# Cogito2012/OpenTAL

Hardware: AMD Instinct MI355X
Metric: clips/sec training step, 256-frame THUMOS14 clips (higher is better)
Workload: dtype bf16

## Files before the change

include/opental_hip.h:

```cpp
#ifndef OPENTAL_HIP_H
#define OPENTAL_HIP_H

#include <stdint.h>
#include <stddef.h>

#ifdef __cplusplus
extern "C" {
#endif

#define OTAL_ABI_VERSION 26

#define OTAL_E_NULL      (-1)
#define OTAL_E_SHAPE     (-2)
#define OTAL_E_ODD_C     (-3)
#define OTAL_E_BATCH     (-4)
#define OTAL_E_DTYPE     (-5)
#define OTAL_E_LEVELS    (-6)
#define OTAL_E_UNSUPPORTED (-7)

#define OTAL_F32  0
#define OTAL_BF16 1
#define OTAL_F16  2
#define OTAL_F64  3

#define OTAL_MAX_LEVELS 8

int otal_abi_version(void);
const char* otal_error_string(int code);
int otal_set_option(const char* name, int value);
int otal_get_option(const char* name, int dflt);
int otal_stream_wait(void* waiter, void* signaler);

int otal_bmp_fwd(const void* in, const float* seg, void* out,
                 int B, int C, int T, int N, int seg_batch, int dtype, void* stream);

int otal_bmp_bwd(const void* grad_out, const void* in, const float* seg, void* grad_in,
                 int B, int C, int T, int N, int seg_batch, int compat_ref_stride,
                 int dtype, void* stream);

int otal_bmp_fwd_levels(const void* in, const float* seg, void* out,
                        int B, int C, int nlev, const int* t_start, const int* n_start,
                        int dtype, void* stream);
int otal_bmp_bwd_levels(const void* grad_out, const void* in, const float* seg, void* grad_in,
                        int B, int C, int nlev, const int* t_start, const int* n_start,
                        int dtype, void* stream);

int otal_conv_half_storage(const int* geom, const int64_t* strides, int mode, int precision);
size_t otal_conv_workspace_bytes(const int* geom, int mode);

int otal_conv_fwd(const int* geom, const int64_t* strides, const float* x, const float* w,
                  const float* scale, const float* shift, float* y, int relu, int precision,
                  const void* prologue, void* ws, size_t ws_bytes, void* stream);

int otal_conv_dgrad(const int* geom, const int64_t* strides, const float* dy, const float* wt_packed,
                    float* dx, int accumulate, const float* out_mask, const float* out_scale,
                    int precision, const void* prologue, void* ws, size_t ws_bytes, void* stream);

int otal_conv_wgrad(const int* geom, const int64_t* strides, const float* x, const float* dy,
                    float* dw, int accumulate, int precision, const void* prologue, void* ws, size_t ws_bytes,
                    void* stream);

int otal_conv_fwd_pair(const int* geom, const int64_t* strides, const float* const* x, const float* const* w,
                       const float* const* scale, const float* const* shift, float* const* y, int relu, int precision,
                       const void* const* prologue, void* ws, size_t ws_bytes, void* stream);
int otal_conv_dgrad_pair(const int* geom, const int64_t* strides, const float* const* dy, const float* const* w,
                         float* const* dx, int precision, const void* const* prologue, void* ws, size_t ws_bytes, void* stream);
int otal_conv_wgrad_pair(const int* geom, const int64_t* strides, const float* const* x, const float* const* dy,
                         float* const* dw, int precision, void* ws, size_t ws_bytes, void* stream);

size_t otal_conv_prologue_bytes(const int* geom, const int64_t* strides, int mode, int precision);
size_t otal_conv_prologue_desc_bytes(void);
int otal_conv_prologue(const int* geom, const int64_t* strides, int mode, const float* w, int precision, void* region,
                       size_t region_bytes, void* host_desc, void* stream);
int otal_conv_prologue_batch(int n, const void* device_descs, const int* device_starts, int total_blocks, void* stream);

int otal_conv_defer_reduces(int on);
size_t otal_conv_deferred_end(void);
int otal_conv_deferred_count(void);
int otal_conv_flush_reduces(void* stream);

const char* otal_conv_last_kernel(void);

int otal_conv_pack_wt(const float* w, float* wt, int Cout, int Cin, int kvol, void* stream);

int otal_gn_relu_fwd(const float* x, const float* gamma, const float* beta, float* y, float* stats,
                     int B, int C, int T, int G, float eps, int relu, int nlev, const int* lev, void* stream);
int otal_gn_relu_bwd(const float* dy, int64_t dy_batch_stride, const float* x, const float* gamma, const float* beta,
                     const float* stats, float* dx, float* partial, int B, int C, int T, int G,
                     int relu, int nlev, const int* lev, void* stream);
int otal_gn_relu_fwd_pair(const float* const* x, const float* const* gamma, const float* const* beta, float* const* y,
                          float* const* stats, int B, int C, int T, int G, float eps, int relu, int nlev, const int* lev,
                          void* stream);
int otal_gn_relu_bwd_pair(const float* const* dy, const int64_t* dy_batch_stride, const float* const* x,
                          const float* const* gamma, const float* const* beta, const float* const* stats, float* const* dx,
                          float* const* partial, int B, int C, int T, int G, int relu, int nlev, const int* lev, void* stream);
int otal_sum_partials(int n_items, const float* const* partial, float* const* dst0, float* const* dst1,
                      float* const* dst2, const int* channels, const int* batches, void* stream);

const char* otal_layer_last_kernel(void);

int otal_maxpool3d_fwd(const int* geom, const int64_t* strides, const float* x, float* y,
                       unsigned char* argtap, void* stream);
int otal_maxpool3d_bwd(const int* geom, const int64_t* strides, const float* dy,
                       const unsigned char* argtap, float* dx, int accumulate,
                       const float* out_mask, const float* out_scale, void* stream);
size_t otal_maxpool3d_signbits_bytes(const int* geom, const int64_t* strides);
int otal_maxpool3d_fwd_signbits(const int* geom, const int64_t* strides, const float* x, float* y,
                                unsigned char* argtap, unsigned char* signbits, void* stream);
int otal_maxpool3d_bwd_signbits(const int* geom, const int64_t* strides, const float* dy, const unsigned char* argtap,
                                float* dx, int accumulate, const unsigned char* signbits, const float* out_scale,
                                void* stream);
int otal_maxpool3d_fwd_signbits_h(const int* geom, const int64_t* strides, const void* x_bf16, float* y,
                                  unsigned char* argtap, unsigned char* signbits, void* stream);
int otal_maxpool3d_bwd_signbits_h(const int* geom, const int64_t* strides, const float* dy, const unsigned char* argtap,
                                  void* dx_bf16, const unsigned char* signbits, const float* out_scale, void* stream);
int otal_maxpool3d_fwd_io(const int* geom, const int64_t* strides, const void* x, void* y, unsigned char* argtap,
                          unsigned char* signbits, int io, void* stream);
int otal_maxpool3d_bwd_io(const int* geom, const int64_t* strides, const void* dy, const unsigned char* argtap, void* dx,
                          int accumulate, const void* out_mask, const float* out_scale, const unsigned char* signbits, int io,
                          void* stream);
int otal_convert_storage(const void* src, int64_t src_bs, int64_t src_cs, void* dst, int64_t dst_bs, int64_t dst_cs,
                         int to_bf16, int B, int C, int P, void* stream);

int otal_head_outputs_fwd(int n_items, const int* channels, const int* modes, const float* const* raw, float* const* out,
                          float* const* unct, const float* scales, int B, int N, int nlev, const int* lev,
                          const float* level_strides, void* stream);
int otal_head_outputs_bwd(int n_items, const int* channels, const int* modes, const float* const* raw,
                          const float* const* out, const float* const* unct, const float* const* dout,
                          const float* const* dunct, float* const* draw, const float* scales, float* dscales, int B,
                          int N, int nlev, const int* lev, const float* level_strides, void* stream);

int otal_boundary_bce(const float* x, int64_t x_batch_stride, int64_t x_channel_stride, const float* mask,
                      int64_t mask_batch_stride, int64_t mask_row_stride, int mask_row0, int mask_step, float* terms,
                      float* dx, int B, int C, int T, void* stream);

int otal_boundary_finish(int n, const float* const* terms, const float* weights, const int* T, int B, float* out2, void* stream);
int otal_boundary_scale(int n, const float* const* dx, float* const* out, const float* weights, const int* C, const int* T,
                        int B, const float* g_start, const float* g_end, void* stream);

int otal_proposal_windows(const float* loc, float* seg, float* frame_seg, int B, int nlev,
                          const int* lev, float frame_num, void* stream);

int otal_decode_clips(const float* loc, const float* prop_loc, const float* priors, const float* conf,
                      const float* prop_conf, const float* center, const float* act, const float* prop_act,
                      const float* offsets, const float* fps, float* seg, float* score, float* unct,
                      float* actn, unsigned char* flag, int nclips, int A, int K, float clip_length,
                      float conf_thresh, void* stream);
int otal_decode_clips_ex(const float* loc, const float* prop_loc, const float* priors, const float* conf,
                         const float* prop_conf, const float* center, const float* act, const float* prop_act,
                         const float* offsets, const float* fps, float* seg, float* score, float* unct,
                         float* actn, unsigned char* flag, int nclips, int A, int K, float clip_length,
                         float conf_thresh, int score_fn, int first_class, void* stream);
int otal_decode_clips_ev(const float* loc, const float* prop_loc, const float* priors, const float* conf,
                         const float* prop_conf, const float* center, const float* act, const float* prop_act,
                         const float* offsets, const float* fps, float* seg, float* score, float* unct,
                         float* actn, unsigned char* flag, int nclips, int A, int K, float clip_length,
                         float conf_thresh, int score_fn, int first_class, int evidence, void* stream);
int otal_softnms_classes(const float* seg, const float* score, const float* unct, const float* actn,
                         const unsigned char* flag, const int* clip_start, int nvideos, int max_clips,
                         int A, int K, float sigma, int top_k, float score_threshold, float* out,
                         int* counts, int* out_index, int out_cols, void* stream);
size_t otal_softnms_scratch_bytes(int total_clips, int max_clips, int A, int K);
int otal_softnms_classes_ws(const float* seg, const float* score, const float* unct, const float* actn,
                            const unsigned char* flag, const int* clip_start, int nvideos, int max_clips,
                            int A, int K, float sigma, int top_k, float score_threshold, float* out,
                            int* counts, int* out_index, int out_cols, void* scratch, size_t scratch_bytes,
                            int total_clips, void* stream);
int otal_detection_table(const float* rows, const int* counts, const double* durations, int V, int K, int top_k, int cols,
                         int drop_empty, int scoring, int* video, int* cls, double* seg, float* sup, double* known,
                         int* list_start, void* stream);
int otal_anchor_stats(const float* loc, const float* conf, const float* prop_conf, const float* center, const float* act,
                      const float* prop_act, const float* priors, const float* gt, const unsigned char* gvalid, int B, int K,
                      int C, int G, float clip_length, float overlap_thresh, int os_head, int n_known, int target,
                      int score_bins, int grad_bins, long long* hist_score, long long* hist_grad, int* label, float* value,
                      float* grad, void* stream);
int otal_anchor_stats_ev(const float* loc, const float* conf, const float* prop_conf, const float* center, const float* act,
                         const float* prop_act, const float* priors, const float* gt, const unsigned char* gvalid, int B,
                         int K, int C, int G, float clip_length, float overlap_thresh, int os_head, int n_known, int target,
                         int score_bins, int grad_bins, long long* hist_score, long long* hist_grad, int* label,
                         float* value, float* grad, int evidence, void* stream);

int otal_openmax_dist(const float* feat, int N, int rows_per_batch, int64_t sb, int64_t sr, int64_t sc, const float* mav,
                      int K, int D, const int* labels, float* dist, void* stream);
int otal_openmax_class_means(const float* feat, int N, int rows_per_batch, int64_t sb, int64_t sr, int64_t sc,
                             const int* labels, int K, int D, float* means, int* counts, void* stream);
int otal_openmax_probs(const float* logits, int64_t ldl, const float* feat, int N, int rows_per_batch, int64_t sb, int64_t sr,
                       int64_t sc, const float* mav, const float* wb, int K, int D, int R, float* probs, void* stream);
int otal_decode_clips_openmax(const float* loc, const float* prop_loc, const float* priors, const float* conf,
                              const float* prop_conf, const float* center, const float* offsets, const float* fps,
                              const float* feat, const float* prop_feat, const int64_t* feat_strides,
                              const int64_t* prop_feat_strides, const float* mav, const float* mav_prop, const float* wb,
                              const float* wb_prop, float* seg, float* score, float* unknown, unsigned char* flag,
                              int nclips, int A, int C, int first_class, int D, int R, int refined_feature,
                              float clip_length, float conf_thresh, void* stream);

int otal_openmax_dist_wide(const float* feat, int N, int rows_per_batch, int64_t sb, int64_t sr, int64_t sc, const float* mav,
                           int K, int D, const int* labels, float* dist, void* stream);
int otal_openmax_probs_wide(const float* logits, int64_t ldl, const float* feat, int N, int rows_per_batch, int64_t sb,
                            int64_t sr, int64_t sc, const float* mav, const float* wb, int K, int D, int R, float* probs,
                            void* stream);
int otal_decode_clips_openmax_wide(const float* loc, const float* prop_loc, const float* priors, const float* conf,
                                   const float* prop_conf, const float* center, const float* offsets, const float* fps,
                                   const float* feat, const float* prop_feat, const int64_t* feat_strides,
                                   const int64_t* prop_feat_strides, const float* mav, const float* mav_prop, const float* wb,
                                   const float* wb_prop, float* seg, float* score, float* unknown, unsigned char* flag,
                                   int nclips, int A, int C, int first_class, int D, int R, int refined_feature,
                                   float clip_length, float conf_thresh, void* stream);

int otal_head_convs_supported(int n_heads, int n_inputs, const int* in_idx, const int* cout, const int* ksize, int B, int C, int N);
int otal_head_convs_fwd(int n_heads, int n_inputs, const int* in_idx, const int* cout, const int* ksize,
                        const float* const* x, const float* const* w, const float* const* bias, float* const* y, int B, int C,
                        int N, int nlev, const int* lev, void* stream);
int otal_head_convs_bwd(int n_heads, int n_inputs, const int* in_idx, const int* cout, const int* ksize,
                        const float* const* x, const float* const* w, const float* const* dy, float* const* dx,
                        float* const* dw, float* const* db, int B, int C, int N, int nlev, const int* lev, void* stream);
int otal_head_convs_bwd_parts(int n_heads, int n_inputs, const int* in_idx, const int* cout, const int* ksize,
                        const float* const* x, const float* const* w, const float* const* dy, float* const* dx,
// ... 116 lines not shown
```

opental_amd/common/ops.py:

```python
import bisect
import ctypes
import os
import warnings
from typing import NamedTuple

import torch

from .. import _lib as L
from .conv_geom import make_geom

_WORKSPACE = {}
WORKSPACE_BYTES = 192 << 20
WORKSPACE_TOTAL = 512 << 20

CONV_PROFILE = None

CONV_PRECISION = 0
HALF_STORAGE = os.environ.get("OTAL_HALF_STORAGE", "1") != "0"
HALF_ACT_DIRECT = os.environ.get("OTAL_HALF_ACT_DIRECT", "0") != "0"
HALF_CHAIN = os.environ.get("OTAL_HALF_CHAIN", "1") != "0"


def _prof_begin():
    if CONV_PROFILE is None:
# ... 527 lines not shown

def _prologue(mode, ga, sa, pkey, w, prec):
    c = STEP.prologues
    if c is None or not (prec & 1):
        return None
    wp = 0
    if mode != 2:
        wp = w.data_ptr()
        r = c.persistent_range
        if r is None or not (r[0] <= wp < r[1]):
            return None
    reg = c.region(mode, ga, sa, (wp, pkey, prec), w, prec)
    if reg is None:
        return None
    return L.ptr(reg)


_PLANS = {}


def _plan(mode, xs, ys, Cout, k, s, levels, spatial_valid, xname, yname):
    key = (mode, xs.shape, xs.stride(), ys.shape, ys.stride(), Cout, k, s, levels, spatial_valid, xs.dtype, ys.dtype,
           xs.device, ys.device)
    plan = _PLANS.get(key)
    if plan is None:
        x5, y5 = _as5(xs), _as5(ys)
        B, Cin, Ti, Hi, Wi = x5.shape
        g, outn = _make_geom(B, Cin, Cout, (Ti, Hi, Wi), k, s, levels, spatial_valid)
        if tuple(y5.shape) != (B, Cout) + outn:
            raise RuntimeError(f"{yname} has shape {tuple(y5.shape)}, expected {(B, Cout) + outn}")
        _check(x5, xname, x5.dtype)
        _check(y5, yname, y5.dtype)
        ga, sa = _geom_arrays(g, x5, y5)
        plan = (g, ga, sa, (mode, tuple(g), _bs(x5), _bs(y5)), (tuple(x5.shape), _bs(x5)))
        if len(_PLANS) > 4096:
            _PLANS.clear()
        _PLANS[key] = plan
    return plan


def _out_positions(x, Cout, k, s, levels, spatial_valid):
    x5 = _as5(x)
    B, Cin, Ti, Hi, Wi = x5.shape
    return _make_geom(B, Cin, Cout, (Ti, Hi, Wi), k, s, levels, spatial_valid)[1]


def half_storage_ok(mode, x_shape, cout, k, s, both=False):
    if not (HALF_STORAGE and int(CONV_PRECISION) & 1) or len(x_shape) != 5:
        return False
    k, s = _k3(k), _k3(s)
    B, Cin, Ti, Hi, Wi = x_shape
    g, outn = _make_geom(B, Cin, cout, (Ti, Hi, Wi), k, s, None, False)
    ga = (ctypes.c_int * len(g))(*g)
    P = outn[0] * outn[1] * outn[2]
    sa = (ctypes.c_int64 * 4)(Cin * Ti * Hi * Wi, Ti * Hi * Wi, cout * P, P)
    return bool(L.lib().otal_conv_half_storage(ga, sa, int(mode), int(CONV_PRECISION) | (12 if both else 0)))


def conv_forward(x, w, k, s, scale=None, shift=None, relu=False, spatial_valid=False, levels=None, out=None, half_out=False):
    k, s = _k3(k), _k3(s)
    if levels is not None:
        levels = tuple(levels)
    Cout = w.shape[0]
    if x.dtype == torch.bfloat16:
        return _conv_forward_half(x, w, k, s, scale, shift, relu, spatial_valid, levels, out)
    if out is None:
        outn = _out_positions(x, Cout, k, s, levels, spatial_valid)
        out = torch.empty((x.shape[0], Cout) + (outn if x.dim() == 5 else outn[:1]),
                          dtype=torch.bfloat16 if half_out else x.dtype, device=x.device)
    if out.dtype != (torch.bfloat16 if half_out else torch.float32) or x.dtype != torch.float32:
        raise RuntimeError("conv_forward: float32 tensors (bfloat16 y with half_out)")
    g, ga, sa, pkey, _ = _plan(0, x, out, Cout, k, s, levels, spatial_valid, "x", "y")
    if not w.is_contiguous():
        raise RuntimeError("weights must be contiguous")
    wsp, wsn = _ws_args(x.device)
    ev = _prof_begin()
    prec = int(CONV_PRECISION)
    pre = _prologue(0, ga, sa, pkey, w, prec)
    L.check(L.lib().otal_conv_fwd(ga, sa, L.ptr(x), L.ptr(w), _opt(scale), _opt(shift), L.ptr(out), int(relu),
                                  prec | (4 if half_out else 0), pre, wsp, wsn, L.stream()),
            "otal_conv_fwd")
    _prof_end(ev, "fwd", g)
    return out


def _conv_forward_half(x, w, k, s, scale, shift, relu, spatial_valid, levels, out):
    Cout = w.shape[0]
    if out is None:
        outn = _out_positions(x, Cout, k, s, levels, spatial_valid)
        out = torch.empty((x.shape[0], Cout) + (outn if x.dim() == 5 else outn[:1]), dtype=torch.bfloat16, device=x.device)
    if out.dtype != torch.bfloat16 or not (int(CONV_PRECISION) & 1):
        raise RuntimeError("conv_forward: a bfloat16 x needs a bfloat16 y and the bf16-operand mode")
    g, ga, sa, pkey, _ = _plan(0, x, out, Cout, k, s, levels, spatial_valid, "x", "y")
    if not w.is_contiguous():
        raise RuntimeError("weights must be contiguous")
    wsp, wsn = _ws_args(x.device)
    ev = _prof_begin()
    prec = int(CONV_PRECISION)
    pre = _prologue(0, ga, sa, pkey, w, prec)
    L.check(L.lib().otal_conv_fwd(ga, sa, L.ptr(x), L.ptr(w), _opt(scale), _opt(shift), L.ptr(out), int(relu),
                                  prec | 12, pre, wsp, wsn, L.stream()), "otal_conv_fwd (bf16 tensors)")
    _prof_end(ev, "fwd", g)
    return out


def pack_wt(w):
    Cout, Cin = w.shape[0], w.shape[1]
    kvol = w[0, 0].numel()
    wt = torch.empty((Cin, Cout, kvol), dtype=w.dtype, device=w.device)
    L.check(L.lib().otal_conv_pack_wt(L.ptr(w), L.ptr(wt), Cout, Cin, kvol, L.stream()), "otal_conv_pack_wt")
    return wt


def conv_dgrad(dy, w, x_shape, k, s, spatial_valid=False, levels=None, out=None,
               accumulate=False, wt=None, out_mask=None, out_scale=None):
    k, s = _k3(k), _k3(s)
    if levels is not None:
        levels = tuple(levels)
    Cout = w.shape[0]
    if out is None:
        if accumulate:
            raise RuntimeError("accumulate needs an existing buffer")
        out = torch.empty(tuple(x_shape), dtype=dy.dtype, device=dy.device)
    elif tuple(out.shape) != tuple(x_shape):
        raise RuntimeError(f"conv_dgrad: out has shape {tuple(out.shape)}, expected {tuple(x_shape)}")
    half = dy.dtype == torch.bfloat16
    if out.dtype != dy.dtype or not (half or dy.dtype == torch.float32):
        raise RuntimeError("conv_dgrad: float32 tensors, or bfloat16 dy / dx / out_mask together")
    if half and (accumulate or not (int(CONV_PRECISION) & 1)):
        raise RuntimeError("conv_dgrad: bfloat16 tensors need the bf16-operand mode and a plain store")
    g, ga, sa, pkey, xlay = _plan(1, out, dy, Cout, k, s, levels, spatial_valid, "dx", "dy")
    prec = int(CONV_PRECISION)
    if wt is None:
        wt = w if w.is_contiguous() else w.contiguous()
        prec |= 2
    wsp, wsn = _ws_args(dy.device)
    ev = _prof_begin()
    if out_mask is not None:
        m5 = _as5(out_mask)
        if (tuple(m5.shape), _bs(m5)) != xlay or out_mask.dtype != dy.dtype:
            raise RuntimeError("out_mask must share dx's shape, layout and dtype")
    pre = _prologue(1, ga, sa, pkey, wt, prec) if (prec & 2) else None
    if half:
        prec |= 12 | (16 if out_mask is not None else 0)
    L.check(L.lib().otal_conv_dgrad(ga, sa, L.ptr(dy), L.ptr(wt), L.ptr(out),
                                    int(accumulate), _opt(out_mask), _opt(out_scale), prec, pre,
                                    wsp, wsn, L.stream()),
            "otal_conv_dgrad")
    _prof_end(ev, "dgrad", g)
    return out


def is_full_collapse(x_shape, k, s, spatial_valid):
    return (spatial_valid and len(x_shape) == 5 and tuple(x_shape[3:]) == tuple(k[1:]) and k[0] == 1
            and tuple(s) == (1, 1, 1))


def conv_dgrad_collapse(dy, w, x_shape):
    B, Cin, T, H, W = x_shape
    Cout = w.shape[0]
    wa = w.detach().reshape(1, Cout, Cin * H * W)
    dyt = dy.reshape(B, Cout, T).permute(0, 2, 1).reshape(B * T, Cout, 1).contiguous()
    dxp = conv_forward(wa, dyt, 1, 1)
    return dxp.view(B, T, Cin, H, W).permute(0, 2, 1, 3, 4)


# ... 168 lines not shown
def conv_wgrad_pair(xs, dys, w_shape, k, s, levels=None, outs=(None, None)):
    k, s = _k3(k), _k3(s)
    if levels is not None:
        levels = tuple(levels)
    if not PAIR_LAUNCHES or not (int(CONV_PRECISION) & 1) or not _same_layout(xs[0], xs[1]) or not _same_layout(dys[0], dys[1]):
        return None
    if xs[0].dtype != torch.float32 or dys[0].dtype != torch.float32:
        return None
    Cout = w_shape[0]
    g, ga, sa, pkey, _ = _plan(2, xs[0], dys[0], Cout, k, s, levels, False, "x", "dy")
    outs = [o if o is not None else torch.empty(tuple(w_shape), dtype=torch.float32, device=xs[0].device) for o in outs]
    if not (outs[0].is_contiguous() and outs[1].is_contiguous()):
        return None
    st = STEP
    if st.defer and st.defer_owner is not None and st.defer_owner[0] != st.ws_index:
        flush_reduces()
    wsp, wsn = _ws_args(xs[0].device)
    ev = _prof_begin()
    rc = L.lib().otal_conv_wgrad_pair(ga, sa, _pp(*xs), _pp(*dys), _pp(*outs), int(CONV_PRECISION), wsp, wsn, L.stream())
    if rc == L.E_UNSUPPORTED:
        return None
    L.check(rc, "otal_conv_wgrad_pair")
    if st.defer:
        _after_wgrad(xs[0].device)
    _prof_end(ev, "wgrad", g, 2)
    return outs


def gn_relu_forward_pair(xs, gammas, betas, groups=32, eps=1e-5, relu=True, levels=None, outs=None):
    if not PAIR_LAUNCHES or not _same_layout(xs[0], xs[1]) or not xs[0].is_contiguous():
        return None
    L.require_device(*xs, *gammas, *betas)
    B, C, T = xs[0].shape
    nlev, lev = _lev_arg(levels)
    stats = [torch.empty((B, groups, nlev, 2), dtype=torch.float32, device=x.device) for x in xs]
    if outs is not None:
        st0, st1 = _dest_strides(outs[0], B, C, T), _dest_strides(outs[1], B, C, T)
        if st0 != st1:
            return None
        rc = L.lib().otal_gn_relu_fwd_pair_to(_pp(*xs), _pp(*gammas), _pp(*betas), _pp(*outs), ctypes.c_int64(st0[0]),
                                              ctypes.c_int64(st0[1]), _pp(*stats), B, C, T, groups, ctypes.c_float(eps), int(relu),
                                              nlev, lev, L.stream())
        if rc == L.E_UNSUPPORTED:
            return None
        L.check(rc, "otal_gn_relu_fwd_pair_to")
        return list(zip(outs, stats))
    ys = [torch.empty_like(x) for x in xs]
    rc = L.lib().otal_gn_relu_fwd_pair(_pp(*xs), _pp(*gammas), _pp(*betas), _pp(*ys), _pp(*stats), B, C, T, groups,
                                       ctypes.c_float(eps), int(relu), nlev, lev, L.stream())
    if rc == L.E_UNSUPPORTED:
        return None
    L.check(rc, "otal_gn_relu_fwd_pair")
    return list(zip(ys, stats))


def _lev_arg(levels):
    if levels is None or len(levels) <= 2:
        return 1, None
    return len(levels) - 1, L.int_array(list(levels))


def _dest_strides(out, B, C, T):
    if tuple(out.shape) != (B, C, T) or out.dtype != torch.float32 or not out.is_cuda or (T > 1 and out.stride(2) != 1):
        raise RuntimeError("gn_relu_forward: `out` must be a float32 (B,C,T) GPU tensor with dense positions")
    cs = out.stride(1) if C > 1 else T
    return (out.stride(0) if B > 1 else cs * C), cs


def gn_relu_forward(x, gamma, beta, groups=32, eps=1e-5, relu=True, levels=None, out=None):
    L.require_device(x, gamma, beta)
    B, C, T = x.shape
    nlev, lev = _lev_arg(levels)
    stats = torch.empty((B, groups, nlev, 2), dtype=torch.float32, device=x.device)
    if out is not None:
        bs, cs = _dest_strides(out, B, C, T)
        L.check(L.lib().otal_gn_relu_fwd_to(L.ptr(x), L.ptr(gamma), L.ptr(beta), L.ptr(out), ctypes.c_int64(bs), ctypes.c_int64(cs),
                                            L.ptr(stats), B, C, T, groups, ctypes.c_float(eps), int(relu), nlev, lev, L.stream()),
                "otal_gn_relu_fwd_to")
        return out, stats
    y = torch.empty_like(x)
    L.check(L.lib().otal_gn_relu_fwd(L.ptr(x), L.ptr(gamma), L.ptr(beta), L.ptr(y), L.ptr(stats), B, C, T, groups,
                                     ctypes.c_float(eps), int(relu), nlev, lev, L.stream()), "otal_gn_relu_fwd")
    return y, stats


def pyramid_merge_forward(p0, p1, total, up):
    L.require_device(p0, p1)
    B, C, t0 = p0.shape
    if tuple(p1.shape) != (B, C, t0 // 2):
        raise RuntimeError("pyramid_merge_forward: p1 must have half of p0's positions")
    packed = torch.empty((B, C, total), dtype=torch.float32, device=p0.device)
    frame = torch.empty((B, C, t0 * up), dtype=torch.float32, device=p0.device)
    L.check(L.lib().otal_pyramid_merge_fwd(L.ptr(p0), L.ptr(p1), L.ptr(packed), L.ptr(frame), B, C, t0, total, up, L.stream()),
            "otal_pyramid_merge_fwd")
    return packed, frame


def pyramid_merge_backward(da, db, dframe, dnext, t0, up):
    L.require_device(da, dframe)
    B, C, T = da.shape
    dp0 = torch.empty((B, C, t0), dtype=torch.float32, device=da.device)
    dp1 = torch.empty((B, C, t0 // 2), dtype=torch.float32, device=da.device)
    for t in (db, dnext):
        if t is not None:
            L.require_device(t)
    L.check(L.lib().otal_pyramid_merge_bwd(L.ptr(da), _opt(db), L.ptr(dframe), _opt(dnext), L.ptr(dp0), L.ptr(dp1), B, C, t0, T, up,
                                           L.stream()), "otal_pyramid_merge_bwd")
    return dp0, dp1


def gn_relu_backward(dy, x, gamma, beta, stats, groups=32, relu=True, levels=None, bias=None):
    B, C, T = x.shape
    if dy.dim() != 3 or tuple(dy.shape) != (B, C, T) or dy.stride(2) != 1 or dy.stride(1) != T or dy.stride(0) < C * T:
        dy = dy.contiguous()
    L.require_device(x, gamma, beta, stats)
    if not dy.is_cuda:
        raise RuntimeError("opental_amd ops run on the GPU only")
    nlev, lev = _lev_arg(levels)
    dx = torch.empty_like(x)
    partial = torch.empty((B, 3, C), dtype=torch.float32, device=x.device)
    L.check(L.lib().otal_gn_relu_bwd(L.ptr(dy), ctypes.c_int64(dy.stride(0)), L.ptr(x), L.ptr(gamma), L.ptr(beta), L.ptr(stats),
                                     L.ptr(dx), L.ptr(partial), B, C, T, groups, int(relu), nlev, lev, L.stream()),
            "otal_gn_relu_bwd")
    return (dx,) + _gn_sums(partial, gamma, beta, bias, C, B)


def _gn_sums(partial, gamma, beta, bias, C, B):
    s = STEP
    if s.pending_sums is not None and bias is not None and s.slots is not None:
        slots = [s.slots.take(t) for t in (gamma, beta, bias)]
        if all(sl is not None for sl in slots):
            s.pending_sums.append((partial, tuple(sl.data_ptr() for sl in slots), C, B))
            return slots[0], slots[1], slots[2]
        for t, sl in zip((gamma, beta, bias), slots):
            if sl is not None:
                s.slots.release(t)
    red = partial.sum(0)
    return red[0], red[1], red[2]


def gn_relu_backward_pair(dys, xs, gammas, betas, stats, groups=32, relu=True, levels=None, biases=(None, None)):
    if not PAIR_LAUNCHES or not _same_layout(xs[0], xs[1]):
        return None
    B, C, T = xs[0].shape
    dys = list(dys)
    for i in range(2):
        dy = dys[i]
        if dy.dim() != 3 or tuple(dy.shape) != (B, C, T) or dy.stride(2) != 1 or dy.stride(1) != T or dy.stride(0) < C * T:
            dys[i] = dy.contiguous()
        if not dys[i].is_cuda:
            raise RuntimeError("opental_amd ops run on the GPU only")
    L.require_device(*xs, *gammas, *betas, *stats)
    nlev, lev = _lev_arg(levels)
    dxs = [torch.empty_like(x) for x in xs]
    partials = [torch.empty((B, 3, C), dtype=torch.float32, device=x.device) for x in xs]
    rc = L.lib().otal_gn_relu_bwd_pair(_pp(*dys), (ctypes.c_int64 * 2)(dys[0].stride(0), dys[1].stride(0)), _pp(*xs), _pp(*gammas),
                                       _pp(*betas), _pp(*stats), _pp(*dxs), _pp(*partials), B, C, T, groups, int(relu), nlev, lev,
                                       L.stream())
    if rc == L.E_UNSUPPORTED:
        return None
    L.check(rc, "otal_gn_relu_bwd_pair")
    return [(dxs[i],) + _gn_sums(partials[i], gammas[i], betas[i], biases[i], C, B) for i in range(2)]


def flush_pending_sums():
    items = STEP.pending_sums
# ... 240 lines not shown
    @staticmethod
    def backward(ctx, *gs):
        (grads,) = ctx.saved_tensors
        B, K, C = ctx.dims
        A = B * K
        gs = [None if g is None else g.contiguous() for g in gs]
        out = torch.empty(4 * A + 2 * A * C + 3 * A, dtype=torch.float32, device=grads.device)
        g7 = (ctypes.c_void_p * 7)(*[None if g is None else g.data_ptr() for g in gs])
        L.check(L.lib().otal_detection_loss_bwd(L.ptr(grads), g7, L.ptr(out), B, K, C, L.stream()), "otal_detection_loss_bwd")
        o = 0
        def take(n, shape):
            nonlocal o
            v = out[o:o + n].view(shape)
            o += n
            return v
        d_loc, d_pl = take(2 * A, (B, K, 2)), take(2 * A, (B, K, 2))
        d_conf, d_pconf = take(A * C, (B, K, C)), take(A * C, (B, K, C))
        d_cen, d_act, d_pact = take(A, (B, K)), take(A, (B, K)), take(A, (B, K))
        heads = tuple(d if there else None for d, there in zip((d_loc, d_conf, d_pl, d_pconf, d_cen, d_act, d_pact), ctx.heads))
        return heads + (None,) * (len(ctx.needs_input_grad) - len(heads))


class DetectionLossFunction(_FusedLossFunction):
    ENTRIES = {'plain': 'otal_detection_loss', 'ex': 'otal_detection_loss_ex', 'ev': 'otal_detection_loss_ev'}
    TERMS = 7

    @staticmethod
    def c_args(call, state, B, K, C, G):
        args = [L.ptr(state), B, K, C, G, *_cf(call.clip_length, call.overlap_thresh), int(call.ibm_active), int(call.num_bins),
                *_cf(call.momentum), int(call.iou_aware), int(call.cls_mode), *_cf(call.focal_alpha)]
        if call.entry != 'plain':
            args += [int(call.reweight), *_cf(call.rw_gamma)]
        if call.entry == 'ev':
            args += [int(call.evidence), int(call.loss_type)]
        return args, L.lib().otal_detection_loss_scratch_floats(B, K)


class AnetDetectionLossFunction(_FusedLossFunction):
    ENTRIES = {'anet_ex': 'otal_detection_loss_anet_ex', 'anet_ev': 'otal_detection_loss_anet_ev'}
    TERMS = 7

    @staticmethod
    def c_args(call, state, B, K, C, G):
        nlev = len(call.level_bounds)
        lbs = (ctypes.c_float * (2 * nlev))(*[float(v) for row in call.level_bounds for v in row])
        args = [B, K, C, G, *_cf(call.clip_length, call.overlap_thresh), lbs, nlev, int(call.ibm_active), *_cf(call.ibm_coeff),
                int(call.iou_aware), *_cf(call.act_weight, call.act_margin), int(call.cls_mode), *_cf(call.focal_alpha)]
        if call.entry == 'anet_ev':
            args += [int(call.evidence), int(call.loss_type)]
        return args, 8 * B


class RPLDetectionLossFunction(_FusedLossFunction):
    ENTRIES = {'rpl': 'otal_detection_loss_rpl'}
    TERMS = 5

    @staticmethod
    def c_args(call, state, B, K, C, G):
        args = [B, K, C, G, *_cf(call.clip_length, call.overlap_thresh), int(bool(call.gcpl)),
                *_cf(call.temperature, call.weight_pl, call.radius)]
        return args, L.lib().otal_detection_loss_scratch_floats(B, K)


_SLOT_INDEX = {}


def _adjacent_view(ts):
    if not ts or any(t is None or t.numel() != 1 or t.dtype != torch.float32 for t in ts):
        return None
    base = ts[0]
    st = base.untyped_storage().data_ptr()
    if any(t.untyped_storage().data_ptr() != st or t.data_ptr() != base.data_ptr() + 4 * i for i, t in enumerate(ts)):
        return None
    return base.detach().as_strided((len(ts),), (1,), base.storage_offset())


class HeadOutputsFunction(torch.autograd.Function):

    @staticmethod
    def forward(ctx, levels, level_strides, modes, *tensors):
        nlev_ = len(levels) - 1
        ctx.scale_params = tensors[:nlev_]
        scales = _adjacent_view(tensors[:nlev_])
        if scales is None:
            scales = torch.cat([t.detach().reshape(1) for t in tensors[:nlev_]])
        raws = [r.contiguous() for r in tensors[nlev_:]]
        L.require_device(scales, *raws)
        B, _, N = raws[0].shape
        n = len(raws)
        outs = [torch.empty((B, N, r.shape[1]), dtype=torch.float32, device=r.device) for r in raws]
        uncts = [torch.empty((B, N), dtype=torch.float32, device=raws[0].device) if m >= 2 else None for m in modes]
        VP = ctypes.c_void_p * n
        arr = lambda ts: VP(*[None if t is None else t.data_ptr() for t in ts])
        strides = None if level_strides is None else (ctypes.c_float * len(level_strides))(*level_strides)
        meta = (L.int_array([r.shape[1] for r in raws]), L.int_array(list(modes)), len(levels) - 1, L.int_array(list(levels)), strides, B, N, n)
        L.check(L.lib().otal_head_outputs_fwd(n, meta[0], meta[1], arr(raws), arr(outs), arr(uncts), L.ptr(scales), B, N, meta[2],
                                              meta[3], strides, L.stream()), "otal_head_outputs_fwd")
        ctx.meta, ctx.modes = meta, tuple(modes)
        ctx.save_for_backward(scales, *raws, *outs, *[u for u in uncts if u is not None])
        return tuple(outs) + tuple(u for u in uncts if u is not None)

    @staticmethod
    def backward(ctx, *grads):
        chans, modes_a, nlev, lev, strides, B, N, n = ctx.meta
        saved = ctx.saved_tensors
        scales, raws, outs, us = saved[0], saved[1:1 + n], saved[1 + n:1 + 2 * n], list(saved[1 + 2 * n:])
        uncts, dunct, k = [], [], 0
        for m in ctx.modes:
            if m >= 2:
                uncts.append(us[k]); dunct.append(grads[n + k]); k += 1
            else:
                uncts.append(None); dunct.append(None)
        douts = [None if g is None else g.contiguous() for g in grads[:n]]
        dunct = [None if g is None else g.contiguous() for g in dunct]
        draws = [torch.empty_like(r) for r in raws]
        VP = ctypes.c_void_p * n
        arr = lambda ts: VP(*[None if t is None else t.data_ptr() for t in ts])

        def launch(dscales):
            L.check(L.lib().otal_head_outputs_bwd(n, chans, modes_a, arr(raws), arr(outs), arr(uncts), arr(douts), arr(dunct), arr(draws),
                                                  L.ptr(scales), L.ptr(dscales), B, N, nlev, lev, strides, L.stream()),
                    "otal_head_outputs_bwd")
        want = all(ctx.needs_input_grad[3:3 + nlev])
        slots = [grad_slot(p) if want else None for p in ctx.scale_params]
        direct = _adjacent_view(slots) if all(sl is not None for sl in slots) else None
        if direct is not None:
            direct.zero_()
            launch(direct)
            return (None, None, None) + tuple(slots) + tuple(draws)
        dscales = torch.zeros_like(scales)
        launch(dscales)
        if all(sl is not None for sl in slots):
            key = tuple(sl.data_ptr() for sl in slots)
            idx = _SLOT_INDEX.get(key)
            if idx is None:
                flat = STEP.slots.grad
                idx = torch.tensor([(sl.data_ptr() - flat.data_ptr()) // 4 for sl in slots], dtype=torch.int64).to(flat.device)
                if len(_SLOT_INDEX) > 64:
                    _SLOT_INDEX.clear()
                _SLOT_INDEX[key] = idx
            STEP.slots.grad.index_copy_(0, idx, dscales)
            return (None, None, None) + tuple(slots) + tuple(draws)
        for p, sl in zip(ctx.scale_params, slots):
            if sl is not None:
                STEP.slots.release(p)
        aligned = torch.zeros((nlev, 4), dtype=dscales.dtype, device=dscales.device)
        aligned[:, 0] = dscales
        return (None, None, None) + tuple(aligned[l, :1] for l in range(nlev)) + tuple(draws)


def _hc_meta(heads, n_inputs):
    n = len(heads)
    return (n, n_inputs, L.int_array([h[0] for h in heads]), L.int_array([h[1] for h in heads]), L.int_array([h[2] for h in heads]))


def head_convs_supported(heads, n_inputs, B, C, N):
    if not 1 <= len(heads) <= 8 or not 1 <= n_inputs <= 4:
        return False
    n, ni, idx, co, ks = _hc_meta(heads, n_inputs)
    return bool(L.lib().otal_head_convs_supported(n, ni, idx, co, ks, int(B), int(C), int(N)))


class HeadConvsFunction(torch.autograd.Function):

    @staticmethod
    def forward(ctx, levels, heads, n_inputs, *tensors):
        nh = len(heads)
        xs = [t.contiguous() for t in tensors[:n_inputs]]
        ws = list(tensors[n_inputs:n_inputs + nh])
        bs = list(tensors[n_inputs + nh:n_inputs + 2 * nh])
        L.require_device(*xs, *ws, *[b for b in bs if b is not None])
        B, C, N = xs[0].shape
        spec = [(heads[i][0], int(ws[i].shape[0]), int(heads[i][1])) for i in range(nh)]
        for (j, co, k), w in zip(spec, ws):
            if tuple(w.shape) != (co, C, k) or tuple(xs[j].shape) != (B, C, N) or w.dtype != torch.float32:
                raise RuntimeError("head_convs: weight / input shapes do not match")
        meta = _hc_meta(spec, n_inputs)
        nlev, lev = _lev_arg(levels)
        ys = [torch.empty((B, co, N), dtype=torch.float32, device=xs[0].device) for _, co, _ in spec]
        VP = lambda ts: (ctypes.c_void_p * len(ts))(*[None if t is None else t.data_ptr() for t in ts])
        L.check(L.lib().otal_head_convs_fwd(*meta, VP(xs), VP(ws), VP(bs), VP(ys), B, C, N, nlev, lev, L.stream()),
                "otal_head_convs_fwd")
        ctx.cfg = (meta, nlev, lev, n_inputs, nh, (B, C, N), [b is not None for b in bs])
        ctx.bias_params = bs
        ctx.save_for_backward(*xs, *ws)
        return tuple(ys)

    @staticmethod
    def backward(ctx, *dys):
        meta, nlev, lev, n_inputs, nh, (B, C, N), has_bias = ctx.cfg
        saved = ctx.saved_tensors
        xs, ws = list(saved[:n_inputs]), list(saved[n_inputs:])
        dys = [None if g is None else g.contiguous() for g in dys]
        dxs = [torch.empty_like(x) if ctx.needs_input_grad[3 + j] else None for j, x in enumerate(xs)]
        dws, slots_w, slots_b = [], [], []
        for w in ws:
            slot = grad_slot(w)
            slots_w.append(slot)
            dws.append(slot if slot is not None else torch.empty_like(w))
        dbs = []
        for w, b in zip(ws, ctx.bias_params):
            slot = grad_slot(b) if b is not None else None
            slots_b.append(slot)
            dbs.append(slot if slot is not None else (torch.empty(w.shape[0], dtype=torch.float32, device=w.device) if b is not None else None))
        VP = lambda ts: (ctypes.c_void_p * len(ts))(*[None if t is None else t.data_ptr() for t in ts])
        in_slots = all(s_ is not None for s_ in slots_w) and all(s_ is not None for s_, b in zip(slots_b, ctx.bias_params) if b is not None)
        side = side_wgrads(xs[0].device)
        if side.on and in_slots and STEP.defer_join:
            L.check(L.lib().otal_head_convs_bwd_parts(*meta, VP(xs), VP(ws), VP(dys), VP(dxs), VP(dws), VP(dbs), B, C, N, nlev, lev, 1,
                                                      L.stream()), "otal_head_convs_bwd_parts")
            dst_w, dst_b = [t.detach() for t in dws], [None if t is None else t.detach() for t in dbs]
            side.pending.append(lambda: L.check(L.lib().otal_head_convs_bwd_parts(
                *meta, VP(xs), VP(ws), VP(dys), VP([None] * len(xs)), VP(dst_w), VP(dst_b), B, C, N, nlev, lev, 2, L.stream()),
# ... 47 lines not shown
            side.node_end(True)
        else:
            run(opt(dx), L.ptr(dcen), 3 if dx is not None else 2)
        return dx, dcen


def head_convs(levels, items):
    maps, heads = [], []
    for x, unit in items:
        j = next((i for i, m in enumerate(maps) if m is x), None)
        if j is None:
            j = len(maps)
            maps.append(x)
        conv = unit.conv1d
        k = conv.kernel_size[0]
        if conv.stride[0] != 1 or k not in (1, 3) or x.dim() != 3 or x.dtype != torch.float32 or not x.is_cuda:
            return None
        heads.append((j, k, conv))
    B, C, N = maps[0].shape
    if any(tuple(m.shape) != (B, C, N) for m in maps) or C % 16:
        return None
    if not head_convs_supported([(j, conv.out_channels, k) for j, k, conv in heads], len(maps), B, C, N):
        return None
    return HeadConvsFunction.apply(None if levels is None else tuple(levels), tuple((j, k) for j, k, _ in heads), len(maps),
                                   *maps, *[c.weight for _, _, c in heads], *[c.bias for _, _, c in heads])


HC_MAX_ROWS = 21


def head_convs_mixed(levels, items, run_one):
    wide = [unit.conv1d.out_channels > HC_MAX_ROWS for _, unit in items]
    if not any(wide) or all(wide):
        return None
    small = [it for it, w in zip(items, wide) if not w]
    fused = head_convs(levels, small)
    if fused is None:
        return None
    fused = list(fused)
    return [run_one(x, unit) if w else fused.pop(0) for (x, unit), w in zip(items, wide)]


class BoundaryBCEFunction(torch.autograd.Function):

    @staticmethod
    def forward(ctx, x, mask, row0, step):
        if not (x.is_cuda and mask.is_cuda):
            raise RuntimeError("opental_amd ops run on the GPU only")
        B, C, T = x.shape
        if x.stride(2) != 1 or mask.stride(2) != 1 or x.dtype != torch.float32 or mask.dtype != torch.float32:
            raise RuntimeError("boundary_bce: float32 maps with unit time stride")
        if row0 + 2 > mask.shape[1] or (T - 1) * step >= mask.shape[2]:
            raise RuntimeError("boundary_bce: mask rows / length do not cover the map")
        terms = torch.empty((B, 2, T), dtype=torch.float32, device=x.device)
        dx = torch.empty((B, C, T), dtype=torch.float32, device=x.device)
        L.check(L.lib().otal_boundary_bce(L.ptr(x), ctypes.c_int64(x.stride(0)), ctypes.c_int64(x.stride(1)), L.ptr(mask),
                                          ctypes.c_int64(mask.stride(0)), ctypes.c_int64(mask.stride(1)), int(row0), int(step),
                                          L.ptr(terms), L.ptr(dx), B, C, T, L.stream()), "otal_boundary_bce")
        ctx.save_for_backward(dx)
        ctx.x_shape = tuple(x.shape)
        losses = terms.sum(dim=(0, 2)) / float(B * T)
        return losses[0], losses[1]

    @staticmethod
    def backward(ctx, g_start, g_end):
        (dx,) = ctx.saved_tensors
        B, C, T = ctx.x_shape
        z = dx.new_zeros(())
        g = torch.stack([z if g_start is None else g_start.reshape(()), z if g_end is None else g_end.reshape(())])
        return (dx.view(B, 2, C // 2, T) * g.view(1, 2, 1, 1)).view(B, C, T), None, None, None


class BoundaryLossesFunction(torch.autograd.Function):

    @staticmethod
    def forward(ctx, mask, steps, weights, *xs):
        n = len(xs)
        B = xs[0].shape[0]
        terms, dxs = [], []
        for x, step in zip(xs, steps):
            if not (x.is_cuda and mask.is_cuda) or x.stride(2) != 1 or mask.stride(2) != 1 or x.dtype != torch.float32:
                raise RuntimeError("boundary losses: float32 GPU maps with unit time stride")
            _, C, T = x.shape
            if 2 > mask.shape[1] or (T - 1) * step >= mask.shape[2]:
                raise RuntimeError("boundary losses: mask rows / length do not cover the map")
            t = torch.empty((B, 2, T), dtype=torch.float32, device=x.device)
            dx = torch.empty((B, C, T), dtype=torch.float32, device=x.device)
            L.check(L.lib().otal_boundary_bce(L.ptr(x), ctypes.c_int64(x.stride(0)), ctypes.c_int64(x.stride(1)), L.ptr(mask),
                                              ctypes.c_int64(mask.stride(0)), ctypes.c_int64(mask.stride(1)), 0, int(step),
                                              L.ptr(t), L.ptr(dx), B, C, T, L.stream()), "otal_boundary_bce")
            terms.append(t); dxs.append(dx)
        out = torch.empty(2, dtype=torch.float32, device=xs[0].device)
        wa = (ctypes.c_float * n)(*[float(w) for w in weights])
        VP = lambda ts: (ctypes.c_void_p * n)(*[t.data_ptr() for t in ts])
        L.check(L.lib().otal_boundary_finish(n, VP(terms), wa, L.int_array([t.shape[2] for t in terms]), B, L.ptr(out), L.stream()),
                "otal_boundary_finish")
        ctx.save_for_backward(*dxs)
        ctx.meta = (n, B, [float(w) for w in weights])
        return out[0], out[1]

    @staticmethod
    def backward(ctx, g_start, g_end):
        dxs = ctx.saved_tensors
        n, B, weights = ctx.meta
        outs = [torch.empty_like(d) for d in dxs]
        wa = (ctypes.c_float * n)(*weights)
        VP = lambda ts: (ctypes.c_void_p * n)(*[t.data_ptr() for t in ts])
        gs = [None if g is None else g.contiguous() for g in (g_start, g_end)]
        L.check(L.lib().otal_boundary_scale(n, VP(dxs), VP(outs), wa, L.int_array([d.shape[1] for d in dxs]),
                                            L.int_array([d.shape[2] for d in dxs]), B, _opt(gs[0]), _opt(gs[1]), L.stream()),
                "otal_boundary_scale")
        return (None, None, None) + tuple(outs)


def eval_match(pred_seg, pred_start, gt_seg, gt_start, thresholds):
    L.require_device(pred_seg, pred_start, gt_seg, gt_start, thresholds)
    if pred_seg.dtype != torch.float64 or gt_seg.dtype != torch.float64 or thresholds.dtype != torch.float64 \
            or pred_start.dtype != torch.int32 or gt_start.dtype != torch.int32:
        raise RuntimeError("eval_match: segments and thresholds in float64, offsets in int32")
    if pred_seg.dim() != 2 or pred_seg.shape[1] != 2 or gt_seg.dim() != 2 or gt_seg.shape[1] != 2 \
            or pred_start.dim() != 1 or pred_start.shape != gt_start.shape or pred_start.numel() < 1 or thresholds.dim() != 1:
        raise RuntimeError("eval_match: pred_seg (N, 2), gt_seg (M, 2), pred_start / gt_start (ngroups + 1), thresholds (nthr,)")
    N, ngroups, nthr = pred_seg.shape[0], pred_start.numel() - 1, thresholds.numel()
    out = torch.empty((nthr, N), dtype=torch.int32, device=pred_seg.device)
    nonfinite = torch.zeros(1, dtype=torch.int32, device=pred_seg.device)
    if N == 0 or ngroups == 0:
        return out, nonfinite
    if gt_seg.shape[0] == 0:
        gt_seg = gt_seg.new_zeros((1, 2))
    L.check(L.lib().otal_eval_match(L.ptr(pred_seg), L.ptr(pred_start), L.ptr(gt_seg), L.ptr(gt_start), L.ptr(thresholds),
                                    ngroups, nthr, L.ptr(out), L.ptr(nonfinite), L.stream()), "otal_eval_match")
    return out, nonfinite


def eval_match_labeled(pred_seg, pred_label, pred_start, gt_seg, gt_label, gt_start, thresholds):
    L.require_device(pred_seg, pred_label, pred_start, gt_seg, gt_label, gt_start, thresholds)
    if pred_seg.dtype != torch.float64 or gt_seg.dtype != torch.float64 or thresholds.dtype != torch.float64 \
            or any(t.dtype != torch.int32 for t in (pred_start, gt_start, pred_label, gt_label)):
        raise RuntimeError("eval_match_labeled: segments and thresholds in float64, offsets and labels in int32")
    if pred_seg.dim() != 2 or pred_seg.shape[1] != 2 or gt_seg.dim() != 2 or gt_seg.shape[1] != 2 \
            or pred_start.dim() != 1 or pred_start.shape != gt_start.shape or pred_start.numel() < 1 or thresholds.dim() != 1 \
            or pred_label.shape != pred_seg.shape[:1] or gt_label.shape != gt_seg.shape[:1]:
        raise RuntimeError("eval_match_labeled: pred_seg (N, 2), pred_label (N), gt_seg (M, 2), gt_label (M), "
                           "pred_start / gt_start (ngroups + 1), thresholds (nthr,)")
    N, ngroups, nthr = pred_seg.shape[0], pred_start.numel() - 1, thresholds.numel()
    out = torch.empty((nthr, N), dtype=torch.int32, device=pred_seg.device)
    max_tiou = torch.zeros(N, dtype=torch.float64, device=pred_seg.device)
    nonfinite = torch.zeros(1, dtype=torch.int32, device=pred_seg.device)
    if N == 0 or ngroups == 0:
        return out, max_tiou, nonfinite
    if gt_seg.shape[0] == 0:
        gt_seg, gt_label = gt_seg.new_zeros((1, 2)), gt_label.new_zeros(1)
    L.check(L.lib().otal_eval_match_labeled(L.ptr(pred_seg), L.ptr(pred_label), L.ptr(pred_start), L.ptr(gt_seg), L.ptr(gt_label),
                                            L.ptr(gt_start), L.ptr(thresholds), ngroups, nthr, L.ptr(out), L.ptr(max_tiou),
                                            L.ptr(nonfinite), L.stream()), "otal_eval_match_labeled")
    return out, max_tiou, nonfinite


AP_TILE = 256
AP_MAX_CLASS_ROWS = 2 ** 31 - 1 - AP_TILE


def average_precision(codes, rank_pos, class_start, gt_count, out=None):
    L.require_device(codes, rank_pos, class_start, gt_count)
    if any(t.dtype != torch.int32 for t in (codes, rank_pos, class_start, gt_count)):
        raise RuntimeError("average_precision: codes, rank_pos, class_start and gt_count in int32")
    if codes.dim() != 2 or rank_pos.dim() != 1 or rank_pos.shape[0] != codes.shape[1] or class_start.dim() != 1 \
            or class_start.numel() < 2 or gt_count.dim() != 1 or gt_count.numel() != class_start.numel() - 1:
        raise RuntimeError("average_precision: codes (nthr, N), rank_pos (N), class_start (K + 1), gt_count (K)")
    nthr, N = codes.shape
    K = gt_count.numel()
    if out is None:
        out = torch.empty((nthr, K), dtype=torch.float64, device=codes.device)
    else:
        L.require_device(out)
        if tuple(out.shape) != (nthr, K) or out.dtype != torch.float64:
            raise RuntimeError("average_precision: out must be (nthr, K) float64")
# ... 110 lines not shown
```

opental_amd/csrc/bce.hip:

```cpp
#include "common.h"

namespace {

__global__ __launch_bounds__(256) void boundary_bce_kernel(const float* __restrict__ x, int64_t x_bs, int64_t x_cs,
                                                           const float* __restrict__ mask, int64_t m_bs, int64_t m_rs, int row0,
                                                           int m_step, float* __restrict__ terms, float* __restrict__ dx,
                                                           int B, int C, int T) {
    __shared__ float part[16][17];
    const int tl = threadIdx.x & 15, cg = threadIdx.x >> 4;
    const int t = blockIdx.x * 16 + tl, b = blockIdx.y, h = blockIdx.z;
    const int half = C >> 1;
    const bool live = t < T;
    const float* xp = x + (int64_t)b * x_bs + (int64_t)h * half * x_cs + (live ? t : 0);
    constexpr int BCE_MAXI = 32;
    float th[BCE_MAXI];
    const int nit = live ? (half - cg + 15) / 16 : 0;
    float s = 0.f;
#pragma unroll
    for (int i0 = 0; i0 < BCE_MAXI; i0 += 8) {
        if (i0 >= nit) { for (int u = 0; u < 8; ++u) th[i0 + u] = 0.f; continue; }
        float v[8];
#pragma unroll
        for (int u = 0; u < 8; ++u) v[u] = xp[(int64_t)(cg + 16 * min(i0 + u, max(nit - 1, 0))) * x_cs];
#pragma unroll
        for (int u = 0; u < 8; ++u) {
            th[i0 + u] = tanhf(v[u]);
            if (i0 + u < nit) s += th[i0 + u];
        }
    }
    for (int i = BCE_MAXI; i < nit; ++i) s += tanhf(xp[(int64_t)(cg + 16 * i) * x_cs]);
    part[cg][tl] = s;
    __syncthreads();
    float tot = 0.f;
#pragma unroll
    for (int k = 0; k < 16; ++k) tot += part[k][tl];
    if (!live) return;
    const float m = tot / (float)half;
    const float y = mask[(int64_t)b * m_bs + (int64_t)(row0 + h) * m_rs + (int64_t)t * m_step];
    if (cg == 0) {
        const float lm = fmaxf(logf(m), -100.f), l1m = fmaxf(logf(1.f - m), -100.f);
        terms[((int64_t)b * 2 + h) * T + t] = -(y * lm + (1.f - y) * l1m);
    }
    const float gm = (m - y) / fmaxf(m * (1.f - m), 1e-12f) / ((float)B * (float)T) / (float)half;
    float* dp = dx + ((int64_t)b * C + (int64_t)h * half) * T + t;
#pragma unroll
    for (int i = 0; i < BCE_MAXI; ++i)
        if (i < nit) dp[(int64_t)(cg + 16 * i) * T] = gm * (1.f - th[i] * th[i]);
    for (int i = BCE_MAXI; i < nit; ++i) {
        const float t1 = tanhf(xp[(int64_t)(cg + 16 * i) * x_cs]);
        dp[(int64_t)(cg + 16 * i) * T] = gm * (1.f - t1 * t1);
    }
}


constexpr int BL_MAX = 4;
struct BlItems { int n; const float* terms[BL_MAX]; const float* dx[BL_MAX]; float* out[BL_MAX]; float weight[BL_MAX]; int T[BL_MAX]; int C[BL_MAX]; };

__global__ __launch_bounds__(256) void boundary_finish_kernel(BlItems it, int B, float* __restrict__ out) {
    __shared__ float red[256];
    const int t = threadIdx.x;
    for (int h = 0; h < 2; ++h) {
        float total = 0.f;
        for (int i = 0; i < it.n; ++i) {
            const int T = it.T[i], cnt = B * T;
            const float* __restrict__ src = it.terms[i];
            float acc = 0.f;
            for (int e0 = t; e0 < cnt; e0 += 8 * 256) {
                float v[8];
#pragma unroll
                for (int u = 0; u < 8; ++u) {
                    const int e = min(e0 + u * 256, cnt - 1);
                    const int b = e / T, tt = e - b * T;
                    v[u] = src[((size_t)b * 2 + h) * T + tt];
                }
#pragma unroll
                for (int u = 0; u < 8; ++u)
                    if (e0 + u * 256 < cnt) acc += v[u];
            }
            red[t] = acc;
            __syncthreads();
            if (t < 64) {
                float r = (red[t] + red[t + 128]) + (red[t + 64] + red[t + 192]);
#pragma unroll
                for (int s = 32; s > 0; s >>= 1) r += __shfl_down(r, s, 64);
                if (t == 0) red[0] = r;
            }
            __syncthreads();
            total += it.weight[i] * (red[0] / (float)cnt);
            __syncthreads();
        }
        if (t == 0) out[h] = total;
    }
}

__global__ __launch_bounds__(256) void boundary_scale_kernel(BlItems it, int B, const float* __restrict__ g_start,
                                                             const float* __restrict__ g_end) {
    const int i = blockIdx.y;
    const int T = it.T[i], C = it.C[i];
    const int64_t e = (int64_t)blockIdx.x * 256 + threadIdx.x;
    if (e >= (int64_t)B * C * T) return;
    const int c = (int)((e / T) % C);
    const float g = c < C / 2 ? (g_start ? *g_start : 0.f) : (g_end ? *g_end : 0.f);
    it.out[i][e] = it.dx[i][e] * (it.weight[i] * g);
}

}

extern "C" int otal_boundary_bce(const float* x, int64_t x_batch_stride, int64_t x_channel_stride, const float* mask,
                                 int64_t mask_batch_stride, int64_t mask_row_stride, int mask_row0, int mask_step, float* terms,
                                 float* dx, int B, int C, int T, void* stream) {
    if (!x || !mask || !terms || !dx) return OTAL_E_NULL;
    if (B <= 0 || C <= 0 || T <= 0 || (C & 1) || mask_step <= 0 || mask_row0 < 0) return OTAL_E_SHAPE;
    hipLaunchKernelGGL(boundary_bce_kernel, dim3((T + 15) / 16, B, 2), dim3(256), 0, (hipStream_t)stream, x, x_batch_stride,
                       x_channel_stride, mask, mask_batch_stride, mask_row_stride, mask_row0, mask_step, terms, dx, B, C, T);
    return otal_launch_status();
}

extern "C" int otal_boundary_finish(int n, const float* const* terms, const float* weights, const int* T, int B, float* out2,
                                    void* stream) {
    if (!terms || !weights || !T || !out2) return OTAL_E_NULL;
    if (n < 1 || n > BL_MAX || B <= 0) return OTAL_E_SHAPE;
    BlItems it = {};
    it.n = n;
    for (int i = 0; i < n; ++i) {
        if (!terms[i] || T[i] <= 0) return OTAL_E_SHAPE;
        it.terms[i] = terms[i]; it.weight[i] = weights[i]; it.T[i] = T[i];
    }
    hipLaunchKernelGGL(boundary_finish_kernel, dim3(1), dim3(256), 0, (hipStream_t)stream, it, B, out2);
    return otal_launch_status();
}

extern "C" int otal_boundary_scale(int n, const float* const* dx, float* const* out, const float* weights, const int* C,
                                   const int* T, int B, const float* g_start, const float* g_end, void* stream) {
    if (!dx || !out || !weights || !C || !T) return OTAL_E_NULL;
    if (n < 1 || n > BL_MAX || B <= 0) return OTAL_E_SHAPE;
    BlItems it = {};
    it.n = n;
    int64_t most = 0;
    for (int i = 0; i < n; ++i) {
        if (!dx[i] || !out[i] || T[i] <= 0 || C[i] <= 0 || (C[i] & 1)) return OTAL_E_SHAPE;
        it.dx[i] = dx[i]; it.out[i] = out[i]; it.weight[i] = weights[i]; it.T[i] = T[i]; it.C[i] = C[i];
        const int64_t cnt = (int64_t)B * C[i] * T[i];
        most = cnt > most ? cnt : most;
    }
    hipLaunchKernelGGL(boundary_scale_kernel, dim3((unsigned)((most + 255) / 256), n), dim3(256), 0, (hipStream_t)stream, it, B,
                       g_start, g_end);
    return otal_launch_status();
}
```

opental_amd/csrc/conv_gemm.hip:

```cpp
#include "common.h"
#include "conv_index.h"
#include "conv_select.h"
#include <cstdlib>
#include <cstring>
#include <mutex>
#include <type_traits>

#ifndef OTAL_CONV_PART
#define OTAL_CONV_PART 0
#endif

#include "conv1a_tile.h"
namespace otal_conv {
struct ConvArgs;
__attribute__((visibility("hidden"))) int launch_half(int mode, int kernel, int cw, ConvArgs& a, void* ws, size_t ws_bytes, hipStream_t st);
}

namespace {

constexpr int NT = 256;
enum { EPI_RELU = 1, EPI_ACCUM = 2, NO_STORE = 8, NO_BARRIER = 16, EPI_NPAD8 = 32 };

typedef float f32x16 __attribute__((ext_vector_type(16)));

}
struct otal_conv::ConvArgs {
    ConvGeom g;
    ConvFastDiv fd;
    const float* x;
    const float* w;
    const float* dy;
    float* out;
    const float* scale;
    const float* shift;
    float* slab;
    const float* zero;
    const int2* tab;
    const float* emask;
    const float* escale;
    int M, N, K;
    int splits, k_per_split;
    int flags;
    int a_vec4;
    int prec;
    const int2* ctab;
    const unsigned short* wp;
    unsigned src_bytes;
    unsigned wp_bytes;
    int Kp;
    const int2* ptab;
    unsigned dy_bytes;
    int P;
    int w_natural;
    unsigned out_bytes, slab_bytes;
    const void* pre;
    int half;
    int pair;
    const float* x2;
    const float* dy2;
    float* out2;
    const float* scale2;
    const float* shift2;
    const unsigned short* wp2;
    float* slab2;
    const void* pre2;
    const float* w2;
    int xhalf, mhalf;
};
namespace {
using otal_conv::ConvArgs;

__device__ __attribute__((aligned(16))) float g_zero4[4] = {0.f, 0.f, 0.f, 0.f};

__device__ __forceinline__ float ld_or_zero(const float* base, int64_t off, bool ok) {
    const float* p = ok ? base + off : g_zero4;
    return *p;
}

struct Anchor {
    const float* base;
    unsigned mask;
};
__device__ __forceinline__ Anchor anchor_of_output(const ConvGeom& g, const float* x, const PosDec& o, bool live) {
    const int t0 = o.t * g.st - g.pt, h0 = o.h * g.sh - g.ph, w0 = o.w * g.sw - g.pw;
    int lo, up;
// ... 1640 lines not shown
#endif
namespace {
using otal_conv::DEFER_MAX;
using otal_conv::DeferItem;
using otal_conv::DeferBatch;
using otal_conv::g_defer;

__global__ __launch_bounds__(256) void splitk_reduce_batch_kernel(const DeferBatch b) {
    __shared__ float4 part[3][64];
    int item = 0;
#pragma unroll 1
    while (item + 1 < DEFER_MAX && b.start[item + 1] <= (int)blockIdx.x) ++item;
    const DeferItem& d = b.it[item];
    const int wg = (int)blockIdx.x - b.start[item];
    const int lane = threadIdx.x & 63, q = threadIdx.x >> 6;
    const int64_t base = ((int64_t)wg * 64 + lane) * 4;
    const bool live = base < d.total;
    const int per = (d.splits + 3) / 4;
    const int s_lo = q * per, s_hi = min(d.splits, s_lo + per);
    float4 acc = make_float4(0.f, 0.f, 0.f, 0.f);
    if (live) {
        for (int s0 = s_lo; s0 < s_hi; s0 += 8) {
            float4 tmp[8];
#pragma unroll
            for (int u = 0; u < 8; ++u) {
                const int sidx = min(s0 + u, s_hi - 1);
                tmp[u] = *reinterpret_cast<const float4*>(d.slab + (int64_t)sidx * d.total + base);
            }
#pragma unroll
            for (int u = 0; u < 8; ++u)
                if (s0 + u < s_hi) { acc.x += tmp[u].x; acc.y += tmp[u].y; acc.z += tmp[u].z; acc.w += tmp[u].w; }
        }
    }
    if (q > 0) part[q - 1][lane] = acc;
    __syncthreads();
    if (q > 0 || !live) return;
    const float4 p1 = part[0][lane], p2 = part[1][lane], p3 = part[2][lane];
    float r[4] = {(acc.x + p1.x) + (p2.x + p3.x), (acc.y + p1.y) + (p2.y + p3.y), (acc.z + p1.z) + (p2.z + p3.z), (acc.w + p1.w) + (p2.w + p3.w)};
#pragma unroll
    for (int e = 0; e < 4; ++e) {
        const int64_t idx = base + e;
        float v = r[e];
        int64_t off = idx;
        if (d.flags & EPI_NPAD8) {
            const int m = (int)(idx / d.N), n = (int)(idx - (int64_t)m * d.N);
            if ((n & 7) >= d.kw) continue;
            off = (int64_t)m * ((d.N >> 3) * d.kw) + (n >> 3) * d.kw + (n & 7);
        }
        if (d.flags & EPI_ACCUM) v += d.out[off];
        d.out[off] = v;
    }
}

static int flush_deferred(hipStream_t st) {
    std::lock_guard<std::recursive_mutex> lock(g_defer.mu);
    if (g_defer.n == 0) return 0;
    int blocks = 0;
    for (int i = 0; i <= DEFER_MAX; ++i) {
        g_defer.batch.start[i] = blocks;
        if (i < g_defer.n) blocks += (int)((g_defer.batch.it[i].total + 255) / 256);
    }
    hipLaunchKernelGGL(splitk_reduce_batch_kernel, dim3((unsigned)blocks), dim3(256), 0, st, g_defer.batch);
    g_defer.n = 0;
    return otal_launch_status();
}

template <int MODE, bool H = false>
static int launch_splitk_reduce(const ConvArgs& a, hipStream_t st) {
    static_assert(!(H && MODE == MODE_WGRAD), "weight gradients are fp32");
    const int64_t total = (int64_t)a.M * a.N;
    const bool v4 = (total % 4 == 0) && (((uintptr_t)a.slab & 15) == 0);
    if (MODE == MODE_WGRAD) {
        std::lock_guard<std::recursive_mutex> lock(g_defer.mu);
        g_defer.last_end = 0;
        if (g_defer.on && v4 && total <= (1 << 23)) {
            if (g_defer.n == DEFER_MAX)
                if (int e = flush_deferred(st)) return e;
            DeferItem& d = g_defer.batch.it[g_defer.n++];
            d.slab = a.slab; d.out = a.out; d.total = total; d.splits = a.splits; d.flags = a.flags; d.N = a.N; d.kw = a.g.kw;
            g_defer.last_end = reinterpret_cast<uintptr_t>(a.slab + (int64_t)a.splits * total);
            return 0;
        }
    }
    if (v4 && a.splits >= 16 && total <= (1 << 21)) {
        const int blocks = (int)((total / 4 + 63) / 64);
        hipLaunchKernelGGL((splitk_reduce_tall_kernel<MODE, H>), dim3(blocks), dim3(256), 0, st, a);
        return otal_launch_status();
    }
    const int64_t work = v4 ? total / 4 : total;
    const int blocks = (int)((work + 255) / 256 < 4096 ? (work + 255) / 256 : 4096);
    if (v4) hipLaunchKernelGGL((splitk_reduce_kernel<MODE, 4, H>), dim3(blocks), dim3(256), 0, st, a);
    else hipLaunchKernelGGL((splitk_reduce_kernel<MODE, 1, H>), dim3(blocks), dim3(256), 0, st, a);
    return otal_launch_status();
}

__global__ __launch_bounds__(256) void pack_wt_kernel(const float* __restrict__ w, float* __restrict__ wt,
                                                      int Cout, int Cin, int kvol) {
    const int64_t total = (int64_t)Cout * Cin * kvol;
    for (int64_t idx = (int64_t)blockIdx.x * 256 + threadIdx.x; idx < total; idx += (int64_t)gridDim.x * 256) {
        const int r = (int)(idx % kvol);
        const int64_t q = idx / kvol;
        const int co = (int)(q % Cout), ci = (int)(q / Cout);
        wt[idx] = w[((int64_t)co * Cin + ci) * kvol + r];
    }
}

int fill_geom(ConvGeom& g, const int* d) {
    g.B = d[0]; g.Cin = d[1]; g.Cout = d[2];
    g.Ti = d[3]; g.Hi = d[4]; g.Wi = d[5];
    g.To = d[6]; g.Ho = d[7]; g.Wo = d[8];
    g.kt = d[9]; g.kh = d[10]; g.kw = d[11];
    g.st = d[12]; g.sh = d[13]; g.sw = d[14];
    g.pt = d[15]; g.ph = d[16]; g.pw = d[17];
    g.nlev = d[18];
    for (int i = 0; i <= OTAL_CONV_MAX_LEVELS; ++i) g.lev[i] = d[19 + i];
    const int v[] = {g.B, g.Cin, g.Cout, g.Ti, g.Hi, g.Wi, g.To, g.Ho, g.Wo, g.kt, g.kh, g.kw, g.st, g.sh, g.sw};
    for (int x : v) if (x <= 0) return OTAL_E_SHAPE;
    if (g.pt < 0 || g.ph < 0 || g.pw < 0) return OTAL_E_SHAPE;
    if (g.kt > 8 || g.kh > 8 || g.kw > 8) return OTAL_E_UNSUPPORTED;
    if (g.st > 2 || g.sh > 2 || g.sw > 2) return OTAL_E_UNSUPPORTED;
    if (g.nlev > 1) {
        if (g.nlev > OTAL_CONV_MAX_LEVELS || g.Hi != 1 || g.Wi != 1 || g.st != 1 || g.Ti != g.To) return OTAL_E_LEVELS;
        if (g.lev[0] != 0 || g.lev[g.nlev] != g.Ti) return OTAL_E_LEVELS;
        for (int i = 0; i < g.nlev; ++i) if (g.lev[i + 1] <= g.lev[i]) return OTAL_E_LEVELS;
    }
    if ((int64_t)g.Cin * g.Ti * g.Hi * g.Wi >= (1LL << 31) || (int64_t)g.Cout * g.To * g.Ho * g.Wo >= (1LL << 31) ||
        (int64_t)g.Cout * g.Cin * g.kt * g.kh * g.kw >= (1LL << 31)) return OTAL_E_SHAPE;
    if ((int64_t)g.B * g.To * g.Ho * g.Wo >= (1LL << 31) || (int64_t)g.B * g.Ti * g.Hi * g.Wi >= (1LL << 31) ||
        (int64_t)g.Cin * g.kt * g.kh * g.kw >= (1LL << 31) || (int64_t)g.Cout * g.kt * g.kh * g.kw >= (1LL << 31)) return OTAL_E_SHAPE;
    return 0;
}

static const float* zero_word_address() {
    static const float* z = nullptr;
    if (!z) {
        void* p = nullptr;
        if (hipGetSymbolAddress(&p, HIP_SYMBOL(g_zero4)) == hipSuccess) z = static_cast<const float*>(p);
    }
    return z;
}

template <int MODE>
static void set_epilogue_extents(ConvArgs& a) {
    const ConvGeom& g = a.g;
    int64_t out;
    if (MODE == MODE_FWD) out = 4 * ((int64_t)(g.B - 1) * g.y_bs + (int64_t)(g.Cout - 1) * g.y_cs + conv_out_positions(g));
    else if (MODE == MODE_DGRAD) out = 4 * ((int64_t)(g.B - 1) * g.x_bs + (int64_t)(g.Cin - 1) * g.x_cs + conv_in_positions(g));
    else out = 4 * (int64_t)g.Cout * g.Cin * conv_kvol(g);
    a.out_bytes = (out > 0 && out < (int64_t)0xfffffff0u) ? (unsigned)out : 0u;
    const int64_t slab = 4 * (int64_t)a.splits * a.M * a.N;
    a.slab_bytes = (a.splits > 1 && slab < (int64_t)0xfffffff0u) ? (unsigned)slab : 0u;
}

struct DirectArgs {
    ConvArgs c;
    const unsigned short* wp;
    int C, Ktot;
    unsigned wp_bytes;
};

template <int BM, int MODE, int BNP, int WN, int PX = 48, int MINW = 1, bool XPF2 = false, bool H = false>
__global__ __launch_bounds__(BNP * 2 / WN, MINW) void conv3_direct_kernel(const DirectArgs d) {
    constexpr int DNT = BNP * 2 / WN;
    constexpr int WM = BM / 32, PA = 304, SPAN_MAX = BNP + (H ? 56 : 52);
    constexpr int ESZ = H ? 2 : 4, XV = H ? 8 : 4;
    static_assert(PX == 48 || PX == 32, "position pitch");
    constexpr int A_PIECES = (BM * 18 + DNT - 1) / DNT;
// ... 580 lines not shown
    float* slab = (second ? a.slab2 : a.slab) + (int64_t)split * a.M * a.N;
#pragma unroll
    for (int r = 0; r < 16; ++r) {
        const int co = co0 + mi * 32 + (r & 3) + 8 * (r >> 2) + 4 * (lane >> 5);
        if (co < g.Cout && ci < g.Cin) {
#pragma unroll
            for (int d = 0; d < KT; ++d) slab[(int64_t)co * a.N + ci * KT + d] = acc[d][r];
        }
    }
}

int launch_wgrad1d(ConvArgs& a, void* ws, size_t ws_bytes, hipStream_t st) {
    const int nchunks = wgrad1d_chunks(a.g), units = a.g.B * nchunks;
    const int upw = units >= 8 ? 4 : units >= 4 ? 2 : 1;
    const int splits = (units + upw - 1) / upw;
    const size_t need = ((size_t)splits * a.M * a.N * sizeof(float) + 255) & ~(size_t)255;
    if (!ws || ws_bytes < need * (a.pair ? 2 : 1)) return OTAL_E_UNSUPPORTED;
    a.splits = splits; a.k_per_split = 0; a.slab = reinterpret_cast<float*>(ws);
    if (a.pair) a.slab2 = reinterpret_cast<float*>(reinterpret_cast<char*>(ws) + need);
    const dim3 grid(splits, a.g.Cin / 64, ((a.g.Cout + 63) / 64) * (a.pair ? 2 : 1));
    if (a.g.kt == 1) hipLaunchKernelGGL(conv_wgrad1d_kernel<1>, grid, dim3(256), 0, st, a, nchunks, units, upw);
    else hipLaunchKernelGGL(conv_wgrad1d_kernel<3>, grid, dim3(256), 0, st, a, nchunks, units, upw);
    if (int e = otal_launch_status()) return e;
    if (int e = launch_splitk_reduce<MODE_WGRAD>(a, st)) return e;
    if (a.pair) {
        ConvArgs b = a;
        b.slab = a.slab2; b.out = a.out2;
        return launch_splitk_reduce<MODE_WGRAD>(b, st);
    }
    return 0;
}

static inline int chunk_vector_width(const ConvGeom& g) {
    if (g.st != 1 || g.sh != 1 || g.sw != 1 || g.nlev > 1) return 1;
    if (g.Wo != g.Wi || (g.kw != 1 && g.kw != 3) || g.pw != (g.kw - 1) / 2) return 1;
    if (g.kt == 1 && g.kh == 1 && g.kw == 1 && g.To == g.Ti && g.Ho == g.Hi && conv_out_positions(g) % 4 == 0)
        return 4;
    if (g.Wi % 4 == 0) return 4;
    if (g.Wi % 2 == 0) return 2;
    return 1;
}

template <int MODE>
static void fill_prep_desc(PrepDesc& d, const ConvArgs& a, int2* ctab, unsigned short* wp) {
    const int C = MODE == MODE_FWD ? a.g.Cin : a.g.Cout;
    const bool kwv = MODE == MODE_FWD && (C % 8) != 0;
    const int BMsel = choose_bm(a.M, !kwv);
    d.ctab = ctab; d.wp = reinterpret_cast<unsigned*>(wp); d.wsrc = a.w; d.g = a.g;
    d.M = a.M; d.Mpad = (a.M + BMsel - 1) / BMsel * BMsel; d.C = C; d.kvol = conv_kvol(a.g);
    d.K = a.K; d.Kp = chunk_kp(a.K); d.nchunk = d.Kp / 8 + CHUNK_PAD; d.kwv = kwv ? 1 : 0; d.natural = a.w_natural; d.mode = MODE;
    d.direct = 0;
    d.fh = make_fastdiv((uint32_t)(d.Kp / 2));
    d.fk = make_fastdiv((uint32_t)d.kvol);
}
static inline unsigned prep_blocks(const PrepDesc& d) {
    if (d.direct) {
        const int64_t pairs = (int64_t)d.Mpad * d.C * 27 / 2;
        if (pairs >= (1LL << 31)) return 0;
        const int64_t blocks = (pairs + 256 * PREP_U - 1) / (256 * PREP_U);
        return (unsigned)(blocks < 2048 ? blocks : 2048);
    }
    const int64_t pairs = (int64_t)d.Mpad * (d.Kp / 2);
    if (pairs >= (1LL << 31)) return 0;
    int64_t blocks = (pairs + 256 * PREP_U - 1) / (256 * PREP_U);
    if (d.mode == MODE_DGRAD && d.natural && d.kvol <= PREP_T_KVOL && !d.kwv) blocks = (int64_t)(d.Mpad / 32) * ((d.Kp + 255) / 256);
    if (blocks < (d.nchunk + 255) / 256) blocks = (d.nchunk + 255) / 256;
    return (unsigned)(blocks > 2048 ? 2048 : blocks);
}
static void launch_prep(const PrepDesc& d, hipStream_t st) {
    if (d.direct) {
        if (d.mode == MODE_FWD) hipLaunchKernelGGL((pack_direct_kernel<MODE_FWD>), dim3(prep_blocks(d)), dim3(256), 0, st, d.wp, d.wsrc, d.M, d.Mpad, d.C, d.natural, d.fh);
        else hipLaunchKernelGGL((pack_direct_kernel<MODE_DGRAD>), dim3(prep_blocks(d)), dim3(256), 0, st, d.wp, d.wsrc, d.M, d.Mpad, d.C, d.natural, d.fh);
        return;
    }
    if (d.mode == MODE_FWD) hipLaunchKernelGGL((prep_chunks_kernel<MODE_FWD>), dim3(prep_blocks(d)), dim3(256), 0, st, d);
    else hipLaunchKernelGGL((prep_chunks_kernel<MODE_DGRAD>), dim3(prep_blocks(d)), dim3(256), 0, st, d);
}

#if OTAL_CONV_PART == 1
typedef short v4s16 __attribute__((ext_vector_type(4)));
#include "conv1x1_stream.inc"
#endif

template <int MODE, bool H = false>
int launch_chunked(ConvArgs& a, void* ws, size_t ws_bytes, hipStream_t st) {
    const int C = MODE == MODE_FWD ? a.g.Cin : a.g.Cout;
    const bool kwv = MODE == MODE_FWD && (C % 8) != 0;
    if (H && (kwv || (a.flags & EPI_ACCUM) || conv_in_positions(a.g) != conv_out_positions(a.g))) return OTAL_E_UNSUPPORTED;
    if (kwv) a.K = a.g.Cin * a.g.kt * a.g.kh * 8;
    const int BMpack = choose_bm(a.M, !kwv);
    int BMsel = BMpack;
    if (H && BMsel == 128) BMsel = 96;
    const int tm = (a.M + BMsel - 1) / BMsel, tn = (a.N + 127) / 128;
    a.Kp = chunk_kp(a.K);
    const size_t tb = chunk_tab_bytes(a.K), wb = chunk_wp_bytes(a.M, BMpack, a.K);
    int2* ctab;
    unsigned short* wp;
    if (a.pre) {
        ctab = reinterpret_cast<int2*>(const_cast<void*>(a.pre));
        wp = reinterpret_cast<unsigned short*>(reinterpret_cast<char*>(const_cast<void*>(a.pre)) + tb);
    } else {
        if (!ws || ws_bytes < tb + wb) return OTAL_E_UNSUPPORTED;
        ctab = reinterpret_cast<int2*>(ws);
        wp = reinterpret_cast<unsigned short*>(reinterpret_cast<char*>(ws) + tb);
        PrepDesc d;
        fill_prep_desc<MODE>(d, a, ctab, wp);
        launch_prep(d, st);
        if (int e = otal_launch_status()) return e;
        ws = reinterpret_cast<char*>(ws) + tb + wb;
        ws_bytes -= tb + wb;
    }
    a.ctab = ctab; a.wp = wp;
#if OTAL_CONV_PART == 1
    if constexpr (H) {
        if (conv1x1_stream_eligible(a.g, MODE)) {
            const int e = launch_conv1x1_stream<MODE>(a, wp, wb, (a.M + BMpack - 1) / BMpack * BMpack, st);
            if (e != OTAL_E_UNSUPPORTED) return e;
        }
    }
#endif
    a.src_bytes = (unsigned)gather_extent_bytes(a.g, MODE, H ? 2 : 4);
    a.wp_bytes = (unsigned)wb;
    a.fd = make_conv_fastdiv(a.g);
    int splits = choose_splits(tm * tn, a.Kp);
    if (splits > 1) {
        const size_t need = (size_t)splits * a.M * a.N * sizeof(float);
        if (ws_bytes < need) {
            splits = (int)(ws_bytes / ((size_t)a.M * a.N * sizeof(float)));
            if (splits < 2) splits = 1;
        }
    }
    const int kps = ((a.Kp + splits - 1) / splits + 31) / 32 * 32;
    splits = (a.Kp + kps - 1) / kps;
    a.splits = splits;
    a.k_per_split = kps;
    a.slab = splits > 1 ? (float*)ws : nullptr;
    set_epilogue_extents<MODE>(a);
    const dim3 grid(tn, tm, splits);
    const int cw = chunk_vector_width(a.g);
#define OTAL_LAUNCH_C(BM_, WM_, WN_)                                                                                   \
    do {                                                                                                               \
        if (cw == 4) hipLaunchKernelGGL((conv_gemm_bf16c_kernel<BM_, WM_, WN_, MODE, 4, false, H>), grid, dim3(NT), 0, st, a);   \
        else if (cw == 2) hipLaunchKernelGGL((conv_gemm_bf16c_kernel<BM_, WM_, WN_, MODE, 2, false, H>), grid, dim3(NT), 0, st, a); \
        else hipLaunchKernelGGL((conv_gemm_bf16c_kernel<BM_, WM_, WN_, MODE, 1, false, H>), grid, dim3(NT), 0, st, a);           \
    } while (0)
    if constexpr (MODE == MODE_FWD && !H) {
        if (kwv) {
            if (BMsel == 128) hipLaunchKernelGGL((conv_gemm_bf16c_kernel<128, 2, 2, MODE_FWD, 1, true>), grid, dim3(NT), 0, st, a);
            else if (BMsel == 96) hipLaunchKernelGGL((conv_gemm_bf16c_kernel<96, 3, 1, MODE_FWD, 1, true>), grid, dim3(NT), 0, st, a);
            else if (BMsel == 64) hipLaunchKernelGGL((conv_gemm_bf16c_kernel<64, 2, 1, MODE_FWD, 1, true>), grid, dim3(NT), 0, st, a);
            else hipLaunchKernelGGL((conv_gemm_bf16c_kernel<32, 1, 1, MODE_FWD, 1, true>), grid, dim3(NT), 0, st, a);
        }
    }
    if (kwv) {
    } else if (BMsel == 192) OTAL_LAUNCH_C(192, 6, 1);
    else if (BMsel == 128) { if constexpr (!H) OTAL_LAUNCH_C(128, 2, 2); }
    else if (BMsel == 96) OTAL_LAUNCH_C(96, 3, 1);
    else if (BMsel == 64) OTAL_LAUNCH_C(64, 2, 1);
    else OTAL_LAUNCH_C(32, 1, 1);
#undef OTAL_LAUNCH_C
    if (int e = otal_launch_status()) return e;
    if (splits > 1) {
        return launch_splitk_reduce<MODE, H>(a, st);
    }
    return 0;
}

template <bool H = false>
int launch_wgrad_vector(ConvArgs& a, int cw, void* ws, size_t ws_bytes, hipStream_t st) {
    const bool pair = a.g.sw == 2;
    if (H && pair) return OTAL_E_UNSUPPORTED;
    if (pair) {
        a.N = a.g.Cin * a.g.kt * a.g.kh * 8;
        a.flags |= EPI_NPAD8;
    }
    const int BMsel = choose_bm(a.M);
    const int tm = (a.M + BMsel - 1) / BMsel, tn = (a.N + 127) / 128;
    const size_t tb = ptab_bytes(a.g, cw);
    a.fd = make_conv_fastdiv(a.g);
    a.P = conv_out_positions(a.g);
    a.src_bytes = (unsigned)gather_extent_bytes(a.g, MODE_FWD, H ? 2 : 4);
    a.dy_bytes = (unsigned)gather_extent_bytes(a.g, MODE_DGRAD, H ? 2 : 4);
    int2* ptab;
    if (a.pre) {
        ptab = reinterpret_cast<int2*>(const_cast<void*>(a.pre));
    } else {
        if (!ws || ws_bytes < tb) return OTAL_E_UNSUPPORTED;
        ptab = reinterpret_cast<int2*>(ws);
        const int ngroups = a.K / cw, npad = ngroups + PTAB_PAD;
        hipLaunchKernelGGL(build_pos_table_kernel, dim3((npad + 255) / 256), dim3(256), 0, st, ptab, a.g, a.fd, cw, ngroups, npad);
        if (int e = otal_launch_status()) return e;
        ws = reinterpret_cast<char*>(ws) + tb;
        ws_bytes -= tb;
    }
    a.ptab = ptab;
    int splits = choose_splits(tm * tn, a.K, 1, true);
    if (splits > 1) {
        const size_t need = (size_t)splits * a.M * a.N * sizeof(float);
        if (ws_bytes < need) {
            splits = (int)(ws_bytes / ((size_t)a.M * a.N * sizeof(float)));
            if (splits < 2) splits = 1;
        }
    }
    const int kps = ((a.K + splits - 1) / splits + 31) / 32 * 32;
    splits = (a.K + kps - 1) / kps;
    a.splits = splits;
    a.k_per_split = kps;
    a.slab = splits > 1 ? (float*)ws : nullptr;
    set_epilogue_extents<MODE_WGRAD>(a);
    const dim3 grid(tn, tm, splits);
#define OTAL_LAUNCH_W(BM_, WM_, WN_)                                                                                   \
    do {                                                                                                               \
        if (cw == 8) hipLaunchKernelGGL((conv_wgrad_bf16v_kernel<BM_, WM_, WN_, 8, false, H>), grid, dim3(NT), 0, st, a);        \
        else if (cw == 4) hipLaunchKernelGGL((conv_wgrad_bf16v_kernel<BM_, WM_, WN_, 4, false, H>), grid, dim3(NT), 0, st, a);   \
        else hipLaunchKernelGGL((conv_wgrad_bf16v_kernel<BM_, WM_, WN_, 2, false, H>), grid, dim3(NT), 0, st, a);                \
    } while (0)
    if constexpr (!H) {
        if (pair) {
            if (BMsel == 128) hipLaunchKernelGGL((conv_wgrad_bf16v_kernel<128, 2, 2, 8, true>), grid, dim3(NT), 0, st, a);
            else if (BMsel == 96) hipLaunchKernelGGL((conv_wgrad_bf16v_kernel<96, 3, 1, 8, true>), grid, dim3(NT), 0, st, a);
            else if (BMsel == 64) hipLaunchKernelGGL((conv_wgrad_bf16v_kernel<64, 2, 1, 8, true>), grid, dim3(NT), 0, st, a);
            else hipLaunchKernelGGL((conv_wgrad_bf16v_kernel<32, 1, 1, 8, true>), grid, dim3(NT), 0, st, a);
        }
    }
    if (pair) {
    } else if (BMsel == 192) OTAL_LAUNCH_W(192, 6, 1);
    else if (BMsel == 128) OTAL_LAUNCH_W(128, 2, 2);
    else if (BMsel == 96) OTAL_LAUNCH_W(96, 3, 1);
    else if (BMsel == 64) OTAL_LAUNCH_W(64, 2, 1);
    else OTAL_LAUNCH_W(32, 1, 1);
#undef OTAL_LAUNCH_W
    if (int e = otal_launch_status()) return e;
    if (splits > 1) {
        return launch_splitk_reduce<MODE_WGRAD>(a, st);
    }
    return 0;
}

template <int BM, int BNP, int PX = 48, bool H = false>
constexpr int direct_lds_bytes() { return 2 * BM * 304 + 2 * (BNP + (H ? 56 : 52)) * PX + 16; }
template <int BM, int MODE, bool XPF2 = false, bool H = false>
static int launch_direct512(const DirectArgs& d, dim3 grid, hipStream_t st) {
    constexpr int lds = direct_lds_bytes<BM, 512, 48, H>();
    static bool configured = false;
    if (!configured) {
// ... 163 lines not shown
        return launch_splitk_reduce<MODE>(a, st);
    }
    return 0;
}

template <int MODE>
int launch_kernel(const ConvStep& s, ConvArgs& a, void* ws, size_t ws_bytes, hipStream_t st) {
    if constexpr (MODE == MODE_WGRAD) {
        switch (s.kernel) {
            case CK_CONV1A_WGRAD: return launch_conv1a_wgrad(a, ws, ws_bytes, st);
            case CK_PROJ_WGRAD: return launch_proj_wgrad(a, st);
            case CK_WGRAD_DIRECT: return launch_wgrad_direct(a, ws, ws_bytes, st);
            case CK_WGRAD1X1: return launch_wgrad1x1_wide(a, ws, ws_bytes, st);
            case CK_WGRAD_VECTOR: return launch_wgrad_vector(a, s.cw, ws, ws_bytes, st);
            case CK_WGRAD1D: return launch_wgrad1d(a, ws, ws_bytes, st);
        }
    } else {
        switch (s.kernel) {
            case CK_PROJ: if constexpr (MODE == MODE_FWD) return launch_proj_fwd(a, ws, ws_bytes, st); break;
            case CK_CONV1A: if constexpr (MODE == MODE_FWD) return launch_conv1a_direct(a, ws, ws_bytes, st); break;
            case CK_CONV1D_TILE: return launch_conv1d_tile<MODE>(a, ws, ws_bytes, st);
            case CK_DIRECT: return launch_direct<MODE>(a, ws, ws_bytes, st);
            case CK_CHUNKED: return launch_chunked<MODE>(a, ws, ws_bytes, st);
        }
    }
    if (s.kernel == CK_GENERIC) return launch_generic<MODE>(a, ws, ws_bytes, st);
    return OTAL_E_UNSUPPORTED;
}

thread_local const char* g_last_kernel = "";

template <int MODE>
int launch_mode(ConvArgs& a, int precision, void* ws, size_t ws_bytes, hipStream_t st) {
    ConvQuery q = {};
    q.g = a.g;
    q.mode = MODE;
    q.precision = precision;
    q.accumulate = (a.flags & EPI_ACCUM) ? 1 : 0;
    q.has_mask = a.emask ? 1 : 0;
    q.x = (uintptr_t)a.x; q.w = (uintptr_t)a.w; q.dy = (uintptr_t)a.dy; q.out = (uintptr_t)a.out; q.mask = (uintptr_t)a.emask;
    const ConvPlan p = conv_plan(q);
    const void* pre = a.pre;
    int e = OTAL_E_UNSUPPORTED;
    for (int i = 0; i < p.n; ++i) {
        const ConvStep& s = p.step[i];
        a.pre = conv_step_prologue(s.kernel) == p.prologue ? pre : nullptr;
        e = a.xhalf ? otal_conv::launch_half(MODE, s.kernel, s.cw, a, ws, ws_bytes, st) : launch_kernel<MODE>(s, a, ws, ws_bytes, st);
        if (e == 0) g_last_kernel = conv_kernel_name(s.kernel);
        if (e != OTAL_E_UNSUPPORTED || !s.next) return e;
    }
    return e;
}
#endif

}

#if OTAL_CONV_PART == 0
extern "C" size_t otal_conv_workspace_bytes(const int* geom, int mode) {
    ConvGeom g;
    if (!geom || fill_geom(g, geom)) return 0;
    const int kvol = conv_kvol(g);
    int64_t M, N, K;
    if (mode == MODE_FWD) { M = g.Cout; N = (int64_t)g.B * conv_out_positions(g); K = (int64_t)g.Cin * kvol; }
    else if (mode == MODE_DGRAD) { M = g.Cin; N = (int64_t)g.B * conv_in_positions(g); K = (int64_t)g.Cout * kvol; }
    else {
        M = g.Cout; N = (int64_t)g.Cin * kvol; K = (int64_t)g.B * conv_out_positions(g);
        if (g.sw == 2 && g.kw <= 7) N = (int64_t)g.Cin * g.kt * g.kh * 8;
    }
    const int BMsel = choose_bm((int)M);
    const int BN = 128;
    const int tiles = (int)(((M + BMsel - 1) / BMsel) * ((N + BN - 1) / BN));
    int s = choose_splits(tiles, (int)K, 0);
    if (mode == MODE_WGRAD) { const int sw = choose_splits(tiles, (int)K, 1, true); if (sw > s) s = sw; }
    size_t front = mode == MODE_WGRAD ? ptab_bytes(g, 2) : tab_bytes((int)K);
    if (mode != MODE_WGRAD) {
        const int Kc = mode == MODE_FWD && g.Cin * g.kt * g.kh * 8 > K ? g.Cin * g.kt * g.kh * 8 : (int)K;
        size_t cf = chunk_tab_bytes(Kc) + chunk_wp_bytes((int)M, BMsel, Kc);
        if (M % 192 == 0) { const size_t ct = chunk_tab_bytes(Kc) + chunk_wp_bytes((int)M, 192, Kc); if (ct > cf) cf = ct; }
        if (direct_eligible(g, mode, 1, (int)M)) { const size_t dd = direct_wp_bytes(g, (int)M, mode == MODE_FWD ? g.Cin : g.Cout); if (dd > cf) cf = dd; }
        if (cf > front) front = cf;
    }
    if (mode == MODE_DGRAD) front += align256((size_t)g.Cin * g.Cout * kvol * sizeof(float));
    return front + (s > 1 ? (size_t)(s + 1) * M * N * sizeof(float) : 0);
}

extern "C" int otal_conv_fwd(const int* geom, const int64_t* strides, const float* x, const float* w,
                             const float* scale, const float* shift, float* y, int relu, int precision,
                             const void* prologue, void* ws, size_t ws_bytes, void* stream) {
    g_last_kernel = "";
    if (!geom || !strides || !x || !w || !y) return OTAL_E_NULL;
    ConvArgs a = {};
    if (int e = fill_geom(a.g, geom)) return e;
    a.g.x_bs = strides[0]; a.g.x_cs = strides[1]; a.g.y_bs = strides[2]; a.g.y_cs = strides[3];
    a.x = x; a.w = w; a.out = y; a.scale = scale; a.shift = shift;
    a.M = a.g.Cout; a.N = a.g.B * conv_out_positions(a.g); a.K = a.g.Cin * conv_kvol(a.g);
    a.flags = relu ? EPI_RELU : 0;
    a.prec = (precision & 1) ? 1 : 0;
    a.half = (precision & 4) ? 1 : 0;
    a.xhalf = (precision & 8) ? 1 : 0;
    if ((a.half || a.xhalf) && !a.prec) return OTAL_E_UNSUPPORTED;
    if (a.xhalf && !a.half) return OTAL_E_UNSUPPORTED;
    a.pre = prologue;
    return launch_mode<MODE_FWD>(a, precision, ws, ws_bytes, (hipStream_t)stream);
}

extern "C" int otal_conv_dgrad(const int* geom, const int64_t* strides, const float* dy, const float* wt_packed,
                               float* dx, int accumulate, const float* out_mask, const float* out_scale,
                               int precision, const void* prologue, void* ws, size_t ws_bytes, void* stream) {
    g_last_kernel = "";
    if (!geom || !strides || !dy || !wt_packed || !dx) return OTAL_E_NULL;
    if ((out_mask == nullptr) != (out_scale == nullptr)) return OTAL_E_NULL;
    ConvArgs a = {};
    if (int e = fill_geom(a.g, geom)) return e;
    a.g.x_bs = strides[0]; a.g.x_cs = strides[1]; a.g.y_bs = strides[2]; a.g.y_cs = strides[3];
    a.dy = dy; a.w = wt_packed; a.out = dx;
    if (a.g.st > 2 || a.g.sh > 2 || a.g.sw > 2) return OTAL_E_UNSUPPORTED;
    a.emask = out_mask; a.escale = out_scale;
    a.M = a.g.Cin; a.N = a.g.B * conv_in_positions(a.g); a.K = a.g.Cout * conv_kvol(a.g);
    a.flags = accumulate ? EPI_ACCUM : 0;
    a.prec = (precision & 1) ? 1 : 0;
    a.w_natural = (precision & 2) ? 1 : 0;
    a.half = (precision & 4) ? 1 : 0;
    a.xhalf = (precision & 8) ? 1 : 0;
    a.mhalf = (precision & 16) ? 1 : 0;
    if ((a.half || a.xhalf || a.mhalf) && !a.prec) return OTAL_E_UNSUPPORTED;
    if (a.half != a.xhalf || (a.mhalf && !a.xhalf) || (out_mask && a.xhalf && !a.mhalf)) return OTAL_E_UNSUPPORTED;
    a.pre = prologue;
    return launch_mode<MODE_DGRAD>(a, precision, ws, ws_bytes, (hipStream_t)stream);
}

extern "C" int otal_conv_wgrad(const int* geom, const int64_t* strides, const float* x, const float* dy,
                               float* dw, int accumulate, int precision,
                               const void* prologue, void* ws, size_t ws_bytes, void* stream) {
    g_last_kernel = "";
    if (!geom || !strides || !x || !dy || !dw) return OTAL_E_NULL;
    ConvArgs a = {};
    if (int e = fill_geom(a.g, geom)) return e;
    a.g.x_bs = strides[0]; a.g.x_cs = strides[1]; a.g.y_bs = strides[2]; a.g.y_cs = strides[3];
    a.x = x; a.dy = dy; a.out = dw;
    a.M = a.g.Cout; a.N = a.g.Cin * conv_kvol(a.g); a.K = a.g.B * conv_out_positions(a.g);
    a.flags = accumulate ? EPI_ACCUM : 0;
    a.prec = (precision & 1) ? 1 : 0;
    a.half = (precision & 4) ? 1 : 0;
    a.xhalf = (precision & 8) ? 1 : 0;
    if ((a.half || a.xhalf) && !a.prec) return OTAL_E_UNSUPPORTED;
    if (a.xhalf && !a.half) return OTAL_E_UNSUPPORTED;
    a.pre = prologue;
    return launch_mode<MODE_WGRAD>(a, precision, ws, ws_bytes, (hipStream_t)stream);
}

namespace {
int pair_geom(ConvArgs& a, const int* geom, const int64_t* strides) {
    if (int e = fill_geom(a.g, geom)) return e;
    a.g.x_bs = strides[0]; a.g.x_cs = strides[1]; a.g.y_bs = strides[2]; a.g.y_cs = strides[3];
    a.pair = 1;
    return 0;
}
}

extern "C" int otal_conv_fwd_pair(const int* geom, const int64_t* strides, const float* const* x, const float* const* w,
                                  const float* const* scale, const float* const* shift, float* const* y, int relu, int precision,
                                  const void* const* prologue, void* ws, size_t ws_bytes, void* stream) {
    if (!geom || !strides || !x || !w || !y || !x[0] || !x[1] || !w[0] || !w[1] || !y[0] || !y[1]) return OTAL_E_NULL;
    ConvArgs a = {};
    if (int e = pair_geom(a, geom, strides)) return e;
    a.x = x[0]; a.x2 = x[1]; a.w = w[0]; a.w2 = w[1]; a.out = y[0]; a.out2 = y[1];
// ... 143 lines not shown
```

opental_amd/csrc/gn.hip:

```cpp
#include "common.h"

namespace {

struct GnLevels { int nlev; int lev[OTAL_MAX_LEVELS + 1]; };

__device__ __forceinline__ float wave_sum(float v) {
#pragma unroll
    for (int o = 32; o > 0; o >>= 1) v += __shfl_down(v, o, 64);
    return v;
}

__device__ __forceinline__ float block_sum(float v, float* red, int tid) {
    v = wave_sum(v);
    __syncthreads();
    if ((tid & 63) == 0) red[tid >> 6] = v;
    __syncthreads();
    return red[0] + red[1] + red[2] + red[3];
}

template <typename F>
__device__ __forceinline__ void for_level(int lane, int nlanes, int cpg, int len, F f) {
    if (len >= nlanes) {
        for (int c = 0; c < cpg; ++c)
            for (int t = lane; t < len; t += nlanes) f(c, t);
    } else {
        const int cpl = nlanes / len, cl = lane / len, t = lane - cl * len;
        if (cl < cpl)
            for (int c = cl; c < cpg; c += cpl) f(c, t);
    }
}

__device__ __forceinline__ void stage_map(float* dst, const float* __restrict__ src, int n, int tid) {
    if (((reinterpret_cast<uintptr_t>(src) | (uintptr_t)(n * 4)) & 15) == 0) {
        for (int i = tid; i < (n >> 2); i += 256) reinterpret_cast<float4*>(dst)[i] = reinterpret_cast<const float4*>(src)[i];
    } else {
        for (int i = tid; i < n; i += 256) dst[i] = src[i];
    }
}

struct GnFwdAlt { const float* x; const float* gamma; const float* beta; float* y; float* stats; };
__global__ __launch_bounds__(256) void gn_relu_fwd_kernel(const float* __restrict__ x, const float* __restrict__ gamma,
                                                          const float* __restrict__ beta, float* __restrict__ y,
                                                          float* __restrict__ stats, int C, int T, int G,
                                                          float eps, int relu, GnLevels L, GnFwdAlt alt,
                                                          int64_t y_bs, int64_t y_cs) {
    if (blockIdx.y) { x = alt.x; gamma = alt.gamma; beta = alt.beta; y = alt.y; stats = alt.stats; }
    extern __shared__ __attribute__((aligned(16))) char smem[];
    float* buf = reinterpret_cast<float*>(smem);
    float* red = buf + (size_t)(C / G) * T;
    float* gam = red + 8;
    const int tid = threadIdx.x;
    const int b = blockIdx.x / G, g = blockIdx.x % G;
    const int cpg = C / G;
    float* bet = gam + cpg;
    const int64_t base = ((int64_t)b * C + (int64_t)g * cpg) * T;
    const int64_t ybase = (int64_t)b * y_bs + (int64_t)g * cpg * y_cs;
    const int n = cpg * T;
    float gv = 0.f, bv = 0.f;
    if (tid < cpg) { gv = gamma[g * cpg + tid]; bv = beta[g * cpg + tid]; }
    stage_map(buf, x + base, n, tid);
    if (tid < cpg) { gam[tid] = gv; bet[tid] = bv; }
    __syncthreads();
    if (L.nlev == 1) {
        const int cnt = n;
        float s = 0.f;
        for (int i = tid; i < cnt; i += 256) s += buf[i];
        const float mean = block_sum(s, red, tid) / (float)cnt;
        float q = 0.f;
        for (int i = tid; i < cnt; i += 256) { const float d = buf[i] - mean; q += d * d; }
        const float var = block_sum(q, red, tid) / (float)cnt;
        const float rstd = 1.0f / sqrtf(var + eps);
        if (tid == 0) {
            stats[((int64_t)b * G + g) * 2 + 0] = mean;
            stats[((int64_t)b * G + g) * 2 + 1] = rstd;
        }
        for_level(tid, 256, cpg, T, [&](int c, int t) {
            float v = (buf[c * T + t] - mean) * rstd * gam[c] + bet[c];
            if (relu) v = fmaxf(v, 0.f);
            y[ybase + (int64_t)c * y_cs + t] = v;
        });
        return;
    }
    const int wave = tid >> 6, lane = tid & 63;
#pragma unroll 1
    for (int l = wave; l < L.nlev; l += 4) {
        const int lo = L.lev[l], len = L.lev[l + 1] - lo;
        const int cnt = cpg * len;
        float s = 0.f;
        for_level(lane, 64, cpg, len, [&](int c, int t) { s += buf[c * T + lo + t]; });
        const float mean = __shfl(wave_sum(s), 0, 64) / (float)cnt;
        float q = 0.f;
        for_level(lane, 64, cpg, len, [&](int c, int t) { const float d = buf[c * T + lo + t] - mean; q += d * d; });
        const float var = __shfl(wave_sum(q), 0, 64) / (float)cnt;
        const float rstd = 1.0f / sqrtf(var + eps);
        if (lane == 0) {
            stats[(((int64_t)b * G + g) * L.nlev + l) * 2 + 0] = mean;
            stats[(((int64_t)b * G + g) * L.nlev + l) * 2 + 1] = rstd;
        }
        for_level(lane, 64, cpg, len, [&](int c, int t) {
            float v = (buf[c * T + lo + t] - mean) * rstd * gam[c] + bet[c];
            if (relu) v = fmaxf(v, 0.f);
            y[ybase + (int64_t)c * y_cs + lo + t] = v;
        });
    }
}

struct GnBwdAlt { const float* dy; const float* x; const float* gamma; const float* beta; const float* stats; float* dx; float* partial; int64_t dy_bs; };
struct GnTerms { int n; int Tn[3]; const float* p[3]; int64_t bs[3]; int64_t cs[3]; };
__global__ __launch_bounds__(256) void gn_relu_bwd_kernel(const float* __restrict__ dy, const float* __restrict__ x,
                                                          const float* __restrict__ gamma, const float* __restrict__ beta,
                                                          const float* __restrict__ stats, float* __restrict__ dx,
                                                          float* __restrict__ partial, int C, int T, int G, int relu,
                                                          GnLevels L, int64_t dy_bs, int keep_dx, GnBwdAlt alt, GnTerms terms) {
    if (blockIdx.y) { dy = alt.dy; x = alt.x; gamma = alt.gamma; beta = alt.beta; stats = alt.stats; dx = alt.dx; partial = alt.partial; dy_bs = alt.dy_bs; }
    extern __shared__ __attribute__((aligned(16))) char smem[];
    const int cpg = C / G;
    float* xb = reinterpret_cast<float*>(smem);
    float* gb = xb + (size_t)cpg * T;
    float* dxl = gb + (size_t)cpg * T;
    float* red = dxl + (keep_dx ? (size_t)cpg * T : 0);
    float* gam = red + 8;
    float* bet = gam + cpg;
    const int tid = threadIdx.x;
    const int b = blockIdx.x / G, g = blockIdx.x % G;
    const int64_t base = ((int64_t)b * C + (int64_t)g * cpg) * T;
    const int n = cpg * T;
    float gv = 0.f, bv = 0.f;
    if (tid < cpg) { gv = gamma[g * cpg + tid]; bv = beta[g * cpg + tid]; }
    const int64_t dbase = (int64_t)b * dy_bs + (int64_t)g * cpg * T;
    const bool solo = L.nlev == 1;
    const int wv = tid >> 6, ln = tid & 63;
    const int first = solo ? tid : ln, stride = solo ? 256 : 64;
    constexpr int GN_LPW = 2;
    float2 st_pre[GN_LPW];
#pragma unroll
    for (int k = 0; k < GN_LPW; ++k) {
        const int l = (solo ? 0 : wv) + k * (solo ? 1 : 4);
        st_pre[k] = make_float2(0.f, 0.f);
        if (l < L.nlev) {
            st_pre[k].x = stats[(((int64_t)b * G + g) * L.nlev + l) * 2 + 0];
            st_pre[k].y = stats[(((int64_t)b * G + g) * L.nlev + l) * 2 + 1];
        }
    }
// ... 51 lines not shown
            const float xh = (xb[p] - mean) * rstd;
            float d = gb[p];
            if (relu && !(xh * ga + bet[c] > 0.f)) d = 0.f;
            xb[p] = xh;
            gb[p] = d;
            const float dg = d * ga;
            s1 += dg;
            s2 += dg * xh;
        });
        float m1, m2;
        if (solo) {
            m1 = block_sum(s1, red, tid) / (float)cnt;
            m2 = block_sum(s2, red, tid) / (float)cnt;
        } else {
            m1 = __shfl(wave_sum(s1), 0, 64) / (float)cnt;
            m2 = __shfl(wave_sum(s2), 0, 64) / (float)cnt;
        }
        for_level(first, stride, cpg, len, [&](int c, int t) {
            const int p = c * T + lo + t;
            const float v = rstd * (gb[p] * gam[c] - m1 - xb[p] * m2);
            dx[base + (int64_t)c * T + lo + t] = v;
            if (keep_dx) dxl[p] = v;
        });
    }
    __syncthreads();
    const int wave = tid >> 6, lane = tid & 63;
    for (int c = wave; c < cpg; c += 4) {
        const int ch = g * cpg + c;
        float a0 = 0.f, a1 = 0.f, a2 = 0.f;
        if (keep_dx) {
            for (int t = lane; t < T; t += 64) {
                const float d = gb[c * T + t], xh = xb[c * T + t];
                a0 += d * xh;
                a1 += d;
                a2 += dxl[c * T + t];
            }
        } else {
            for (int t = lane; t < T; t += 64) {
                const float d = gb[c * T + t], xh = xb[c * T + t];
                a0 += d * xh;
                a1 += d;
                a2 += dx[base + (int64_t)c * T + t];
            }
        }
        a0 = wave_sum(a0); a1 = wave_sum(a1); a2 = wave_sum(a2);
        if (lane == 0) {
            float* p = partial + (int64_t)b * 3 * C + ch;
            p[0] = a0; p[C] = a1; p[2 * C] = a2;
        }
    }
}

constexpr size_t LDS_MAX = 160 * 1024;
template <typename K> int allow_large_lds(K kernel, size_t lds, bool& done) {
    if (lds <= 64 * 1024 || done) return 0;
    if (hipFuncSetAttribute(reinterpret_cast<const void*>(kernel), hipFuncAttributeMaxDynamicSharedMemorySize,
                            (int)LDS_MAX) != hipSuccess) { (void)hipGetLastError(); return OTAL_E_UNSUPPORTED; }
    done = true;
    return 0;
}

int fill_levels(GnLevels& L, int T, int nlev, const int* lev) {
    if (nlev <= 1 || !lev) { L.nlev = 1; L.lev[0] = 0; for (int i = 1; i <= OTAL_MAX_LEVELS; ++i) L.lev[i] = T; return 0; }
    if (nlev > OTAL_MAX_LEVELS || lev[0] != 0 || lev[nlev] != T) return OTAL_E_LEVELS;
    L.nlev = nlev;
    for (int i = 0; i <= OTAL_MAX_LEVELS; ++i) L.lev[i] = lev[i <= nlev ? i : nlev];
    for (int i = 0; i < nlev; ++i) if (L.lev[i + 1] <= L.lev[i]) return OTAL_E_LEVELS;
    return 0;
}

}

extern "C" int otal_gn_relu_fwd(const float* x, const float* gamma, const float* beta, float* y, float* stats,
                                int B, int C, int T, int G, float eps, int relu, int nlev, const int* lev,
                                void* stream) {
    g_layer_kernel = "";
    if (!x || !gamma || !beta || !y || !stats) return OTAL_E_NULL;
    if (B <= 0 || C <= 0 || T <= 0 || G <= 0 || C % G) return OTAL_E_SHAPE;
    GnLevels L;
    if (int e = fill_levels(L, T, nlev, lev)) return e;
    const size_t lds = (size_t)(C / G) * T * 4 + 64 + (size_t)(C / G) * 8;
    if (lds > LDS_MAX) return OTAL_E_UNSUPPORTED;
    static bool large_ok = false;
    if (int e = allow_large_lds(gn_relu_fwd_kernel, lds, large_ok)) return e;
    hipLaunchKernelGGL(gn_relu_fwd_kernel, dim3(B * G), dim3(256), lds, (hipStream_t)stream,
                       x, gamma, beta, y, stats, C, T, G, eps, relu, L, GnFwdAlt{}, (int64_t)C * T, (int64_t)T);
    return otal_layer_launched("gn_relu_fwd<single>");
}

extern "C" int otal_gn_relu_fwd_to(const float* x, const float* gamma, const float* beta, float* y, int64_t y_bs, int64_t y_cs,
                                   float* stats, int B, int C, int T, int G, float eps, int relu, int nlev, const int* lev,
                                   void* stream) {
    g_layer_kernel = "";
    if (!x || !gamma || !beta || !y || !stats) return OTAL_E_NULL;
    if (B <= 0 || C <= 0 || T <= 0 || G <= 0 || C % G || y_cs < T || y_bs < 0) return OTAL_E_SHAPE;
    GnLevels L;
    if (int e = fill_levels(L, T, nlev, lev)) return e;
    const size_t lds = (size_t)(C / G) * T * 4 + 64 + (size_t)(C / G) * 8;
    if (lds > LDS_MAX) return OTAL_E_UNSUPPORTED;
    static bool large_ok = false;
    if (int e = allow_large_lds(gn_relu_fwd_kernel, lds, large_ok)) return e;
    hipLaunchKernelGGL(gn_relu_fwd_kernel, dim3(B * G), dim3(256), lds, (hipStream_t)stream,
                       x, gamma, beta, y, stats, C, T, G, eps, relu, L, GnFwdAlt{}, y_bs, y_cs);
    return otal_layer_launched("gn_relu_fwd<single>");
}

extern "C" int otal_gn_relu_fwd_pair(const float* const* x, const float* const* gamma, const float* const* beta, float* const* y,
                                     float* const* stats, int B, int C, int T, int G, float eps, int relu, int nlev,
                                     const int* lev, void* stream) {
    g_layer_kernel = "";
    if (!x || !gamma || !beta || !y || !stats) return OTAL_E_NULL;
    for (int i = 0; i < 2; ++i) if (!x[i] || !gamma[i] || !beta[i] || !y[i] || !stats[i]) return OTAL_E_NULL;
    if (B <= 0 || C <= 0 || T <= 0 || G <= 0 || C % G) return OTAL_E_SHAPE;
    GnLevels L;
    if (int e = fill_levels(L, T, nlev, lev)) return e;
    const size_t lds = (size_t)(C / G) * T * 4 + 64 + (size_t)(C / G) * 8;
    if (lds > 64 * 1024) return OTAL_E_UNSUPPORTED;
    const GnFwdAlt alt = {x[1], gamma[1], beta[1], y[1], stats[1]};
    hipLaunchKernelGGL(gn_relu_fwd_kernel, dim3(B * G, 2), dim3(256), lds, (hipStream_t)stream,
                       x[0], gamma[0], beta[0], y[0], stats[0], C, T, G, eps, relu, L, alt, (int64_t)C * T, (int64_t)T);
    return otal_layer_launched("gn_relu_fwd<pair>");
}

extern "C" int otal_gn_relu_fwd_pair_to(const float* const* x, const float* const* gamma, const float* const* beta,
                                        float* const* y, int64_t y_bs, int64_t y_cs, float* const* stats, int B, int C, int T,
                                        int G, float eps, int relu, int nlev, const int* lev, void* stream) {
    g_layer_kernel = "";
    if (!x || !gamma || !beta || !y || !stats) return OTAL_E_NULL;
    for (int i = 0; i < 2; ++i) if (!x[i] || !gamma[i] || !beta[i] || !y[i] || !stats[i]) return OTAL_E_NULL;
    if (B <= 0 || C <= 0 || T <= 0 || G <= 0 || C % G || y_cs < T || y_bs < 0) return OTAL_E_SHAPE;
    GnLevels L;
    if (int e = fill_levels(L, T, nlev, lev)) return e;
    const size_t lds = (size_t)(C / G) * T * 4 + 64 + (size_t)(C / G) * 8;
    if (lds > 64 * 1024) return OTAL_E_UNSUPPORTED;
    const GnFwdAlt alt = {x[1], gamma[1], beta[1], y[1], stats[1]};
    hipLaunchKernelGGL(gn_relu_fwd_kernel, dim3(B * G, 2), dim3(256), lds, (hipStream_t)stream,
                       x[0], gamma[0], beta[0], y[0], stats[0], C, T, G, eps, relu, L, alt, y_bs, y_cs);
    return otal_layer_launched("gn_relu_fwd<pair>");
}

extern "C" int otal_gn_relu_bwd(const float* dy, int64_t dy_batch_stride, const float* x, const float* gamma, const float* beta,
                                const float* stats, float* dx, float* partial, int B, int C, int T, int G,
                                int relu, int nlev, const int* lev, void* stream) {
    g_layer_kernel = "";
    if (!dy || !x || !gamma || !beta || !stats || !dx || !partial) return OTAL_E_NULL;
    if (B <= 0 || C <= 0 || T <= 0 || G <= 0 || C % G) return OTAL_E_SHAPE;
    if (dy_batch_stride == 0) dy_batch_stride = (int64_t)C * T;
    if (dy_batch_stride < (int64_t)C * T) return OTAL_E_SHAPE;
    GnLevels L;
    if (int e = fill_levels(L, T, nlev, lev)) return e;
    size_t lds = (size_t)(C / G) * T * 12 + 64 + (size_t)(C / G) * 8;
    const int keep_dx = lds <= LDS_MAX;
    if (!keep_dx) lds -= (size_t)(C / G) * T * 4;
    if (lds > LDS_MAX) return OTAL_E_UNSUPPORTED;
    static bool large_ok = false;
    if (int e = allow_large_lds(gn_relu_bwd_kernel, lds, large_ok)) return e;
    hipLaunchKernelGGL(gn_relu_bwd_kernel, dim3(B * G), dim3(256), lds, (hipStream_t)stream,
                       dy, x, gamma, beta, stats, dx, partial, C, T, G, relu, L, dy_batch_stride, keep_dx, GnBwdAlt{}, GnTerms{});
    return otal_layer_launched(keep_dx ? "gn_relu_bwd<single,keep_dx,terms=0>" : "gn_relu_bwd<single,no_keep_dx,terms=0>");
}

extern "C" int otal_gn_relu_bwd_sum(int n_terms, const float* const* dy, const int64_t* dy_bs, const int64_t* dy_cs, const int* dy_T,
                                    const float* x, const float* gamma, const float* beta, const float* stats, float* dx,
                                    float* partial, int B, int C, int T, int G, int relu, int nlev, const int* lev, void* stream) {
    g_layer_kernel = "";
    if (!dy || !dy_bs || !dy_cs || !dy_T || !x || !gamma || !beta || !stats || !dx || !partial) return OTAL_E_NULL;
    if (B <= 0 || C <= 0 || T <= 0 || G <= 0 || C % G || n_terms < 1 || n_terms > 3) return OTAL_E_SHAPE;
    GnTerms tm = {};
    tm.n = n_terms;
    for (int k = 0; k < n_terms; ++k) {
        if (!dy[k]) return OTAL_E_NULL;
        if (dy_T[k] <= 0 || dy_T[k] > T || dy_cs[k] < dy_T[k] || dy_bs[k] < 0) return OTAL_E_SHAPE;
        tm.p[k] = dy[k]; tm.bs[k] = dy_bs[k]; tm.cs[k] = dy_cs[k]; tm.Tn[k] = dy_T[k];
    }
    GnLevels L;
    if (int e = fill_levels(L, T, nlev, lev)) return e;
    size_t lds = (size_t)(C / G) * T * 12 + 64 + (size_t)(C / G) * 8;
    const int keep_dx = lds <= LDS_MAX;
    if (!keep_dx) lds -= (size_t)(C / G) * T * 4;
    if (lds > LDS_MAX) return OTAL_E_UNSUPPORTED;
    static bool large_ok = false;
    if (int e = allow_large_lds(gn_relu_bwd_kernel, lds, large_ok)) return e;
    hipLaunchKernelGGL(gn_relu_bwd_kernel, dim3(B * G), dim3(256), lds, (hipStream_t)stream,
                       dy[0], x, gamma, beta, stats, dx, partial, C, T, G, relu, L, (int64_t)C * T, keep_dx, GnBwdAlt{}, tm);
    static const char* const names[2][3] = {
        {"gn_relu_bwd<single,no_keep_dx,terms=1>", "gn_relu_bwd<single,no_keep_dx,terms=2>", "gn_relu_bwd<single,no_keep_dx,terms=3>"},
        {"gn_relu_bwd<single,keep_dx,terms=1>", "gn_relu_bwd<single,keep_dx,terms=2>", "gn_relu_bwd<single,keep_dx,terms=3>"}};
    return otal_layer_launched(names[keep_dx][n_terms - 1]);
}

extern "C" int otal_gn_relu_bwd_pair(const float* const* dy, const int64_t* dy_batch_stride, const float* const* x,
                                     const float* const* gamma, const float* const* beta, const float* const* stats,
                                     float* const* dx, float* const* partial, int B, int C, int T, int G, int relu, int nlev,
                                     const int* lev, void* stream) {
    g_layer_kernel = "";
    if (!dy || !dy_batch_stride || !x || !gamma || !beta || !stats || !dx || !partial) return OTAL_E_NULL;
    int64_t bs[2];
    for (int i = 0; i < 2; ++i) {
        if (!dy[i] || !x[i] || !gamma[i] || !beta[i] || !stats[i] || !dx[i] || !partial[i]) return OTAL_E_NULL;
        bs[i] = dy_batch_stride[i] ? dy_batch_stride[i] : (int64_t)C * T;
        if (bs[i] < (int64_t)C * T) return OTAL_E_SHAPE;
    }
    if (B <= 0 || C <= 0 || T <= 0 || G <= 0 || C % G) return OTAL_E_SHAPE;
    GnLevels L;
    if (int e = fill_levels(L, T, nlev, lev)) return e;
    size_t lds = (size_t)(C / G) * T * 12 + 64 + (size_t)(C / G) * 8;
    const int keep_dx = lds <= 64 * 1024;
    if (!keep_dx) lds -= (size_t)(C / G) * T * 4;
    if (lds > 64 * 1024) return OTAL_E_UNSUPPORTED;
    const GnBwdAlt alt = {dy[1], x[1], gamma[1], beta[1], stats[1], dx[1], partial[1], bs[1]};
    hipLaunchKernelGGL(gn_relu_bwd_kernel, dim3(B * G, 2), dim3(256), lds, (hipStream_t)stream,
                       dy[0], x[0], gamma[0], beta[0], stats[0], dx[0], partial[0], C, T, G, relu, L, bs[0], keep_dx, alt, GnTerms{});
    return otal_layer_launched(keep_dx ? "gn_relu_bwd<pair,keep_dx,terms=0>" : "gn_relu_bwd<pair,no_keep_dx,terms=0>");
}

namespace {
constexpr int SP_MAX = 32;
struct SumItems { const float* src[SP_MAX]; float* dst[SP_MAX][3]; int C[SP_MAX]; int B[SP_MAX]; };
__global__ __launch_bounds__(256) void sum_partials_kernel(const SumItems it) {
    const int i = blockIdx.y, r = blockIdx.z, c = blockIdx.x * 256 + threadIdx.x;
    const int C = it.C[i], B = it.B[i];
    if (c >= C || !it.dst[i][r]) return;
    const float* p = it.src[i] + (size_t)r * C + c;
    float v[8];
    float s = 0.f;
    for (int b0 = 0; b0 < B; b0 += 8) {
#pragma unroll
        for (int u = 0; u < 8; ++u) v[u] = b0 + u < B ? p[(size_t)(b0 + u) * 3 * C] : 0.f;
#pragma unroll
        for (int u = 0; u < 8; ++u) if (b0 + u < B) s += v[u];
    }
    it.dst[i][r][c] = s;
}
}

extern "C" int otal_sum_partials(int n_items, const float* const* partial, float* const* dst0, float* const* dst1,
                                 float* const* dst2, const int* channels, const int* batches, void* stream) {
    g_layer_kernel = "";
    if (!partial || !dst0 || !dst1 || !dst2 || !channels || !batches) return OTAL_E_NULL;
    if (n_items < 0) return OTAL_E_SHAPE;
    for (int i0 = 0; i0 < n_items; i0 += SP_MAX) {
        SumItems it = {};
        const int n = n_items - i0 < SP_MAX ? n_items - i0 : SP_MAX;
        int cmax = 0;
        for (int i = 0; i < n; ++i) {
            if (!partial[i0 + i] || channels[i0 + i] <= 0 || batches[i0 + i] <= 0) return OTAL_E_SHAPE;
            it.src[i] = partial[i0 + i];
            it.dst[i][0] = dst0[i0 + i]; it.dst[i][1] = dst1[i0 + i]; it.dst[i][2] = dst2[i0 + i];
            it.C[i] = channels[i0 + i]; it.B[i] = batches[i0 + i];
            cmax = channels[i0 + i] > cmax ? channels[i0 + i] : cmax;
        }
        hipLaunchKernelGGL(sum_partials_kernel, dim3((cmax + 255) / 256, n, 3), dim3(256), 0, (hipStream_t)stream, it);
        if (int e = otal_layer_launched("sum_partials")) return e;
    }
    return 0;
}
```

opental_amd/csrc/heads.hip:

```cpp
#include "common.h"
#include "evidence.h"

namespace {

constexpr int MAX_ITEMS = 8;
struct HeadItems {
    int n_items;
    int C[MAX_ITEMS];
    int mode[MAX_ITEMS];
    const float* raw[MAX_ITEMS];
    float* out[MAX_ITEMS];
    float* unct[MAX_ITEMS];
    const float* dout[MAX_ITEMS];
    const float* dunct[MAX_ITEMS];
    float* draw[MAX_ITEMS];
};
struct HeadLevels { int nlev; int lev[OTAL_MAX_LEVELS + 1]; float stride[OTAL_MAX_LEVELS]; };

__device__ __forceinline__ int level_of(const HeadLevels& L, int n) {
    int l = 0;
#pragma unroll
    for (int j = 1; j < OTAL_MAX_LEVELS; ++j)
        if (j < L.nlev && n >= L.lev[j]) l = j;
    return l;
}

__global__ __launch_bounds__(256) void heads_fwd_kernel(HeadItems it, HeadLevels L, const float* __restrict__ scales, int B, int N) {
    const int n = blockIdx.x * 256 + threadIdx.x, b = blockIdx.y, i = blockIdx.z;
    if (n >= N) return;
    const int C = it.C[i], mode = it.mode[i];
    const float* x = it.raw[i] + (size_t)b * C * N + n;
    float* y = it.out[i] + ((size_t)b * N + n) * C;
    if (mode == 1) {
        const int l = level_of(L, n);
        const float s = scales[l], f = L.stride[l];
        for (int c = 0; c < C; ++c) y[c] = expf(x[(size_t)c * N] * s) * f;
        return;
    }
    float sum = 0.f;
    for (int c = 0; c < C; ++c) {
        const float v = x[(size_t)c * N];
        y[c] = v;
        if (mode == 2) sum += expf(fminf(fmaxf(v, -10.f), 10.f)) + 1.f;
        else if (mode > 2) sum += otal_ev::alpha(v, mode - 2);
    }
    if (mode >= 2) it.unct[i][(size_t)b * N + n] = (float)C / sum;
}

__global__ __launch_bounds__(256) void heads_bwd_kernel(HeadItems it, HeadLevels L, const float* __restrict__ scales,
                                                        float* __restrict__ dscales, int B, int N) {
    const int i = blockIdx.z;
    if (i == it.n_items) {
        if (blockIdx.x != 0 || blockIdx.y != 0) return;
        __shared__ float red[256];
        for (int l = 0; l < L.nlev; ++l) {
            float acc = 0.f;
            for (int j = 0; j < it.n_items; ++j) {
                if (it.mode[j] != 1 || !it.dout[j]) continue;
                const int C = it.C[j], t = L.lev[l + 1] - L.lev[l], cnt = B * t * C;
                for (int e = threadIdx.x; e < cnt; e += 256) {
                    const int c = e % C, q = e / C, nn = L.lev[l] + q % t, b = q / t;
                    const size_t o = ((size_t)b * N + nn) * C + c;
                    acc += it.dout[j][o] * it.out[j][o] * it.raw[j][((size_t)b * C + c) * N + nn];
                }
            }
            red[threadIdx.x] = acc;
            __syncthreads();
            for (int s = 128; s > 0; s >>= 1) {
                if (threadIdx.x < s) red[threadIdx.x] += red[threadIdx.x + s];
                __syncthreads();
            }
            if (threadIdx.x == 0) dscales[l] = red[0];
            __syncthreads();
        }
        return;
    }
    const int n = blockIdx.x * 256 + threadIdx.x, b = blockIdx.y;
    if (n >= N) return;
    const int C = it.C[i], mode = it.mode[i];
    float* dx = it.draw[i] + (size_t)b * C * N + n;
    const float* dy = it.dout[i] ? it.dout[i] + ((size_t)b * N + n) * C : nullptr;
    if (mode == 1) {
        const float s = scales[level_of(L, n)];
        const float* y = it.out[i] + ((size_t)b * N + n) * C;
        for (int c = 0; c < C; ++c) dx[(size_t)c * N] = dy ? dy[c] * y[c] * s : 0.f;
        return;
    }
    float coef = 0.f;
    const float* x = it.raw[i] + (size_t)b * C * N + n;
    if (mode >= 2 && it.dunct[i]) {
        const float u = it.unct[i][(size_t)b * N + n];
        coef = -it.dunct[i][(size_t)b * N + n] * u * u / (float)C;
    }
    for (int c = 0; c < C; ++c) {
        float g = dy ? dy[c] : 0.f;
        if (coef != 0.f) {
            const float v = x[(size_t)c * N];
            g += coef * otal_ev::dalpha(v, mode - 2);
        }
        dx[(size_t)c * N] = g;
    }
}

int fill(HeadItems& it, HeadLevels& L, int n_items, const int* channels, const int* modes, int B, int N, int nlev, const int* lev,
         const float* strides) {
    if (n_items < 1 || n_items > MAX_ITEMS || B <= 0 || N <= 0) return OTAL_E_SHAPE;
    if (nlev < 1 || nlev > OTAL_MAX_LEVELS || !lev || lev[0] != 0 || lev[nlev] != N) return OTAL_E_LEVELS;
    it = HeadItems{};
    it.n_items = n_items;
    for (int i = 0; i < n_items; ++i) {
        if (channels[i] <= 0 || modes[i] < 0 || modes[i] > 4) return OTAL_E_SHAPE;
        it.C[i] = channels[i]; it.mode[i] = modes[i];
    }
    L.nlev = nlev;
    for (int i = 0; i <= OTAL_MAX_LEVELS; ++i) L.lev[i] = lev[i <= nlev ? i : nlev];
    for (int i = 0; i < nlev; ++i) if (L.lev[i + 1] <= L.lev[i]) return OTAL_E_LEVELS;
    for (int i = 0; i < OTAL_MAX_LEVELS; ++i) L.stride[i] = (strides && i < nlev) ? strides[i] : 1.f;
    return 0;
}

}

extern "C" int otal_head_outputs_fwd(int n_items, const int* channels, const int* modes, const float* const* raw, float* const* out,
                                     float* const* unct, const float* scales, int B, int N, int nlev, const int* lev,
                                     const float* level_strides, void* stream) {
    if (!channels || !modes || !raw || !out || !unct) return OTAL_E_NULL;
    HeadItems it;
    HeadLevels L;
    if (int e = fill(it, L, n_items, channels, modes, B, N, nlev, lev, level_strides)) return e;
    for (int i = 0; i < n_items; ++i) {
        if (!raw[i] || !out[i] || (modes[i] >= 2 && !unct[i]) || (modes[i] == 1 && !scales)) return OTAL_E_NULL;
        it.raw[i] = raw[i]; it.out[i] = out[i]; it.unct[i] = unct[i];
    }
    hipLaunchKernelGGL(heads_fwd_kernel, dim3((N + 255) / 256, B, n_items), dim3(256), 0, (hipStream_t)stream, it, L, scales, B, N);
    return otal_launch_status();
}

extern "C" int otal_head_outputs_bwd(int n_items, const int* channels, const int* modes, const float* const* raw,
                                     const float* const* out, const float* const* unct, const float* const* dout,
                                     const float* const* dunct, float* const* draw, const float* scales, float* dscales, int B,
                                     int N, int nlev, const int* lev, const float* level_strides, void* stream) {
    if (!channels || !modes || !raw || !out || !unct || !dout || !dunct || !draw) return OTAL_E_NULL;
    HeadItems it;
    HeadLevels L;
    if (int e = fill(it, L, n_items, channels, modes, B, N, nlev, lev, level_strides)) return e;
    bool any_exp = false;
    for (int i = 0; i < n_items; ++i) {
        if (!raw[i] || !out[i] || !draw[i] || (modes[i] >= 2 && !unct[i])) return OTAL_E_NULL;
        it.raw[i] = raw[i]; it.out[i] = const_cast<float*>(out[i]); it.unct[i] = const_cast<float*>(unct[i]);
        it.dout[i] = dout[i]; it.dunct[i] = dunct[i]; it.draw[i] = draw[i];
        any_exp = any_exp || modes[i] == 1;
    }
    if (any_exp && (!scales || !dscales)) return OTAL_E_NULL;
    hipLaunchKernelGGL(heads_bwd_kernel, dim3((N + 255) / 256, B, n_items + (any_exp ? 1 : 0)), dim3(256), 0, (hipStream_t)stream,
                       it, L, scales, dscales, B, N);
    return otal_launch_status();
}
```

opental_amd/thumos14/pyramid_fused.py:

```python
import ctypes

import torch
from torch.autograd import Function

from .. import _lib as L
from ..common import ops
from ..common.i3d_backbone import I3DFeaturesFunction
from ..prop_pooling import boundary_pooling_op as bp

ONE = (1, 1, 1)
K3, K1, S2 = (3, 1, 1), (1, 1, 1), (2, 1, 1)


def _bs_cs(t):
    B, C, T = t.shape
    if T > 1 and t.stride(2) != 1:
        raise RuntimeError("pyramid_fused: positions must be dense")
    cs = t.stride(1) if C > 1 else T
    return (t.stride(0) if B > 1 else cs * C), cs


def _gn_bwd_raw(dy, c, gamma, beta, stats, groups, levels):
    B, C, T = c.shape
    if dy.dim() != 3 or tuple(dy.shape) != (B, C, T) or dy.stride(2) != 1 or dy.stride(1) != T or dy.stride(0) < C * T:
# ... 9 lines not shown
def _gn_bwd_adds(adds, c, gamma, beta, stats, groups, levels):
    B, C, T = c.shape
    n = len(adds)
    dc = torch.empty_like(c)
    partial = torch.empty((B, 3, C), dtype=torch.float32, device=c.device)
    nlev, lev = ops._lev_arg(levels)
    strides = [_bs_cs(t) for t, _ in adds]
    ptrs = (ctypes.c_void_p * n)(*[t.data_ptr() for t, _ in adds])
    I64 = ctypes.c_int64 * n
    L.check(L.lib().otal_gn_relu_bwd_sum(n, ptrs, I64(*[s[0] for s in strides]), I64(*[s[1] for s in strides]),
                                         (ctypes.c_int * n)(*[t.shape[2] if Ta is None else Ta for t, Ta in adds]),
                                         L.ptr(c), L.ptr(gamma), L.ptr(beta), L.ptr(stats), L.ptr(dc), L.ptr(partial),
                                         B, C, T, groups, 1, nlev, lev, L.stream()), "otal_gn_relu_bwd_sum")
    return dc, partial


class _Wgrads:

    def __init__(self, device):
        self.side = ops.side_wgrads(device)
        self.in_slots = True

    def one(self, x, dc, w, k, s, sv=False, levels=None):
        slot = ops.grad_slot(w)
        self.in_slots = self.in_slots and slot is not None
        return self.side.wgrad(x, dc, w.shape, k, s, spatial_valid=sv, levels=levels, out=slot)

    def pair(self, xs, dcs, ws, k, s, levels=None):
        slots = (ops.grad_slot(ws[0]), ops.grad_slot(ws[1]))
        self.in_slots = self.in_slots and slots[0] is not None and slots[1] is not None
        return self.side.wgrad_pair(xs, dcs, ws[0].shape, k, s, levels, slots)


def _conv_gn_pair(xs, ps, k, levels, groups, eps, outs=None):
    ws, bs = (ps[0][0], ps[1][0]), (ps[0][1], ps[1][1])
    cs = ops.conv_forward_pair(xs, ws, k, ONE, bs, levels)
    if cs is None:
        cs = [ops.conv_forward(x, w, k, ONE, shift=b, levels=levels) for x, w, b in zip(xs, ws, bs)]
    r = ops.gn_relu_forward_pair(cs, (ps[0][2], ps[1][2]), (ps[0][3], ps[1][3]), groups, eps, True, levels, outs=outs)
    if r is None:
        r = [ops.gn_relu_forward(c, p[2], p[3], groups, eps, True, levels, out=None if outs is None else outs[i])
             for i, (c, p) in enumerate(zip(cs, ps))]
    return [(cs[i], r[i][0], r[i][1]) for i in range(2)]


def _gn_bwd_pair(dys, cs, ps, stats, groups, levels):
    B, C, T = cs[0].shape
    nlev, lev = ops._lev_arg(levels)
    ok = ops.PAIR_LAUNCHES and all(d.dim() == 3 and d.stride(2) == 1 and d.stride(1) == T and d.stride(0) >= C * T for d in dys)
    if ok:
        dcs = [torch.empty_like(c) for c in cs]
        parts = [torch.empty((B, 3, C), dtype=torch.float32, device=c.device) for c in cs]
        pp = ops._pp
        rc = L.lib().otal_gn_relu_bwd_pair(pp(*dys), (ctypes.c_int64 * 2)(dys[0].stride(0), dys[1].stride(0)), pp(*cs),
                                           pp(ps[0][2], ps[1][2]), pp(ps[0][3], ps[1][3]), pp(*stats), pp(*dcs), pp(*parts),
                                           B, C, T, groups, 1, nlev, lev, L.stream())
        if rc == 0:
            return list(zip(dcs, parts))
        if rc != L.E_UNSUPPORTED:
            L.check(rc, "otal_gn_relu_bwd_pair")
    return [_gn_bwd_raw(dys[i], cs[i], ps[i][2], ps[i][3], stats[i], groups, levels) for i in range(2)]


def _dgrad_pair(dcs, ws, x_shape, k, levels):
    r = ops.conv_dgrad_pair(dcs, ws, x_shape, k, ONE, levels)
    if r is None:
        r = [ops.conv_dgrad(dc, w, x_shape, k, ONE, levels=levels) for dc, w in zip(dcs, ws)]
    return r


class TrunkFunction(Function):

    @staticmethod
    def forward(ctx, cfg, x1, x2, *params):
        lev, up, G, eps = cfg["levels"], cfg["up"], cfg["groups"], cfg["eps"]
        P = [params[4 * i:4 * i + 4] for i in range(13)]
        pyr, dec, lt, ct = P[0:6], P[6:9], P[9:11], P[11:13]
        B = x1.shape[0]
        C = pyr[0][0].shape[0]
        t0, total = lev[1], lev[-1]
        tape = {}
        early = ops.STEP.early_results.pop(x1.data_ptr(), None)
        if early is None:
            c0 = ops.conv_forward(x1, pyr[0][0], cfg["k0"], ONE, shift=pyr[0][1], spatial_valid=True).view(B, C, t0)
            p0, st0 = ops.gn_relu_forward(c0, pyr[0][2], pyr[0][3], G, eps, True, None)
        c1 = ops.conv_forward(x2, pyr[1][0], cfg["k1"], ONE, shift=pyr[1][1], spatial_valid=True).view(B, C, t0 // 2)
        p1, st1 = ops.gn_relu_forward(c1, pyr[1][2], pyr[1][3], G, eps, True, None)
        if early is not None:
            c0, p0, st0, elane = early
            elane.join()
        packed, frame_in = ops.pyramid_merge_forward(p0, p1, total, up)
        tape["proj"] = (c0, st0, c1, st1)
        lane = ops.branch_lane(x1.device)
        use_lane = lane.on
        dtape = []

        def deconv():
            x = frame_in
            for i, k in enumerate((K3, K3, K1)):
                c = ops.conv_forward(x, dec[i][0], k, ONE, shift=dec[i][1])
                y, st = ops.gn_relu_forward(c, dec[i][2], dec[i][3], G, eps, True, None)
                dtape.append((x, c, st, k))
                x = y
            return x
        if use_lane:
            lane.fork()
            with lane:
                frame = deconv()
        ptape = []
        for l in range(2, len(lev) - 1):
            x = packed[:, :, lev[l - 1]:lev[l]]
            c = ops.conv_forward(x, pyr[l][0], K3, S2, shift=pyr[l][1])
            _, st = ops.gn_relu_forward(c, pyr[l][2], pyr[l][3], G, eps, True, None, out=packed[:, :, lev[l]:lev[l + 1]])
            ptape.append((c, st))
        s1 = _conv_gn_pair((packed, packed), (lt[0], ct[0]), K3, lev, G, eps)
        s2 = _conv_gn_pair((s1[0][1], s1[1][1]), (lt[1], ct[1]), K3, lev, G, eps)
        if use_lane:
            lane.join()
        else:
            frame = deconv()
        loc_feat, conf_feat = s2[0][1], s2[1][1]
        ctx.cfg = cfg
        ctx.backbone_joins = getattr(x1.grad_fn, "_forward_cls", None) is I3DFeaturesFunction
        ctx.tape = (tape["proj"], packed, frame_in, dtape, ptape,
                    ((s1[0][0], s1[0][2]), (s1[1][0], s1[1][2]), (s2[0][0], s2[0][2]), (s2[1][0], s2[1][2])),
                    (s1[0][1], s1[1][1]))
        ctx.save_for_backward(x1, x2, *params)
        return loc_feat, conf_feat, frame

    @staticmethod
    def backward(ctx, d_loc, d_conf, d_frame):
        cfg = ctx.cfg
        lev, up, G = cfg["levels"], cfg["up"], cfg["groups"]
        x1, x2 = ctx.saved_tensors[:2]
        params = ctx.saved_tensors[2:]
        P = [params[4 * i:4 * i + 4] for i in range(13)]
        pyr, dec, lt, ct = P[0:6], P[6:9], P[9:11], P[11:13]
        (c0, st0, c1, st1), packed, frame_in, dtape, ptape, tw, (l0, cf0) = ctx.tape
        B, C, t0 = c0.shape
        dev = x1.device
        grads = [None] * len(params)
        WG = _Wgrads(dev)
        sums = []

        def put(i, dw):
            grads[4 * i] = dw
        lane = ops.branch_lane(dev)
        use_lane = lane.on and d_frame is not None
        d_loc, d_conf = d_loc.contiguous(), d_conf.contiguous()
        if d_frame is not None:
            d_frame = d_frame.contiguous()
        d_frame_in = None

        lane_wgrads = []

        hold = []

        def deconv_bwd():
            dy = d_frame
            for i in (2, 1, 0):
                x, c, st, k = dtape[i]
                dc, part = _gn_bwd_raw(dy, c, dec[i][2], dec[i][3], st, G, None)
                sums.append((6 + i, part, B))
                lane_wgrads.append((6 + i, x, dc, dec[i][0], k))
                dy = ops.conv_dgrad(dc, dec[i][0], x.shape, k, ONE)
                hold.append(dy)
            return dy
        if use_lane:
            lane.fork()
            with lane:
                d_frame_in = deconv_bwd()
        r = _gn_bwd_pair((d_loc, d_conf), (tw[2][0], tw[3][0]), (lt[1], ct[1]), (tw[2][1], tw[3][1]), G, lev)
        sums += [(10, r[0][1], B), (12, r[1][1], B)]
        dws = WG.pair((l0, cf0), (r[0][0], r[1][0]), (lt[1][0], ct[1][0]), K3, ONE, lev)
        put(10, dws[0]); put(12, dws[1])
        dmid = _dgrad_pair((r[0][0], r[1][0]), (lt[1][0], ct[1][0]), l0.shape, K3, lev)
        r = _gn_bwd_pair(dmid, (tw[0][0], tw[1][0]), (lt[0], ct[0]), (tw[0][1], tw[1][1]), G, lev)
        sums += [(9, r[0][1], B), (11, r[1][1], B)]
        dws = WG.pair((packed, packed), (r[0][0], r[1][0]), (lt[0][0], ct[0][0]), K3, ONE, lev)
        put(9, dws[0]); put(11, dws[1])
        da, db = _dgrad_pair((r[0][0], r[1][0]), (lt[0][0], ct[0][0]), packed.shape, K3, lev)
        if not use_lane:
            WG.side.flush()
        dnext = None
        for l in range(len(lev) - 2, 1, -1):
            c, st = ptape[l - 2]
            adds = [(da[:, :, lev[l]:lev[l + 1]], None), (db[:, :, lev[l]:lev[l + 1]], None)]
            if dnext is not None:
                adds.append((dnext, None))
            dc, part = _gn_bwd_adds(adds, c, pyr[l][2], pyr[l][3], st, G, None)
            sums.append((l, part, B))
            x = packed[:, :, lev[l - 1]:lev[l]]
            put(l, WG.one(x, dc, pyr[l][0], K3, S2))
            dnext = ops.conv_dgrad(dc, pyr[l][0], x.shape, K3, S2)
        if use_lane:
            lane.join()
# ... 219 lines not shown
```

Baseline: 1013.

## Fuse split-K slab reduction into GroupNorm, batch BCE and head-scale launches

Adds a conv forward path that exposes its split-K partial slabs, so the following GroupNorm+ReLU kernel reduces the slabs itself. This avoids a separate reduce pass and the extra write and read of the conv output. It also merges the per-level boundary BCE launches into one multi-item kernel. Head output kernels now take per-level scale pointers, which removes a torch.cat and a zero-fill of the scale gradients. Together these cut kernel launches and memory traffic, at the cost of more API surface and more special-case paths.

```diff
diff --git a/include/opental_hip.h b/include/opental_hip.h
--- a/include/opental_hip.h
+++ b/include/opental_hip.h
@@ -96,6 +96,14 @@
                           float* const* partial, int B, int C, int T, int G, int relu, int nlev, const int* lev, void* stream);
 int otal_sum_partials(int n_items, const float* const* partial, float* const* dst0, float* const* dst1,
                       float* const* dst2, const int* channels, const int* batches, void* stream);
+
+int otal_conv_fwd_slabs(const int* geom, const int64_t* strides, const float* x, const float* w, const float* scale,
+                        const float* shift, float* y, int relu, int precision, const void* prologue, void* ws, size_t ws_bytes,
+                        void* stream, const float** slab, int* splits);
+int otal_conv_reduce_slabs(const float* slab, int splits, const float* shift, float* out, int B, int C, int T, void* stream);
+int otal_gn_relu_fwd_slabs(const float* slab, int splits, const float* shift, float* xout, const float* gamma,
+                           const float* beta, float* y, int64_t y_bs, int64_t y_cs, float* stats, int B, int C, int T, int G,
+                           float eps, int relu, int nlev, const int* lev, void* stream);
 
 const char* otal_layer_last_kernel(void);
 
@@ -130,9 +138,23 @@
                           const float* const* dunct, float* const* draw, const float* scales, float* dscales, int B,
                           int N, int nlev, const int* lev, const float* level_strides, void* stream);
 
+int otal_head_outputs_fwd_ptrs(int n_items, const int* channels, const int* modes, const float* const* raw, float* const* out,
+                               float* const* unct, const float* const* scale_ptrs, int B, int N, int nlev, const int* lev,
+                               const float* level_strides, void* stream);
+int otal_head_outputs_bwd_ptrs(int n_items, const int* channels, const int* modes, const float* const* raw,
+                               const float* const* out, const float* const* unct, const float* const* dout,
+                               const float* const* dunct, float* const* draw, const float* const* scale_ptrs,
+                               float* const* dscale_ptrs, int B, int N, int nlev, const int* lev, const float* level_strides,
+                               void* stream);
+
 int otal_boundary_bce(const float* x, int64_t x_batch_stride, int64_t x_channel_stride, const float* mask,
                       int64_t mask_batch_stride, int64_t mask_row_stride, int mask_row0, int mask_step, float* terms,
                       float* dx, int B, int C, int T, void* stream);
+
+int otal_boundary_bce_multi(int n, const float* const* x, const int64_t* x_batch_stride, const int64_t* x_channel_stride,
+                            const float* mask, int64_t mask_batch_stride, int64_t mask_row_stride, int mask_row0,
+                            const int* mask_step, float* const* terms, float* const* dx, int B, const int* C, const int* T,
+                            void* stream);
 
 int otal_boundary_finish(int n, const float* const* terms, const float* weights, const int* T, int B, float* out2, void* stream);
 int otal_boundary_scale(int n, const float* const* dx, float* const* out, const float* weights, const int* C, const int* T,
diff --git a/opental_amd/common/ops.py b/opental_amd/common/ops.py
--- a/opental_amd/common/ops.py
+++ b/opental_amd/common/ops.py
@@ -633,6 +633,29 @@
             "otal_conv_fwd")
     _prof_end(ev, "fwd", g)
     return out
+
+
+def conv_forward_slabs(x, w, k, s, shift=None, spatial_valid=False, levels=None):
+    k, s = _k3(k), _k3(s)
+    if levels is not None:
+        levels = tuple(levels)
+    Cout = w.shape[0]
+    if x.dtype != torch.float32:
+        raise RuntimeError("conv_forward_slabs: float32 tensors")
+    outn = _out_positions(x, Cout, k, s, levels, spatial_valid)
+    out = torch.empty((x.shape[0], Cout) + (outn if x.dim() == 5 else outn[:1]), dtype=x.dtype, device=x.device)
+    g, ga, sa, pkey, _ = _plan(0, x, out, Cout, k, s, levels, spatial_valid, "x", "y")
+    if not w.is_contiguous():
+        raise RuntimeError("weights must be contiguous")
+    wsp, wsn = _ws_args(x.device)
+    ev = _prof_begin()
+    prec = int(CONV_PRECISION)
+    pre = _prologue(0, ga, sa, pkey, w, prec)
+    slab, splits = ctypes.c_void_p(), ctypes.c_int(1)
+    L.check(L.lib().otal_conv_fwd_slabs(ga, sa, L.ptr(x), L.ptr(w), None, _opt(shift), L.ptr(out), 0, prec, pre, wsp, wsn,
+                                        L.stream(), ctypes.byref(slab), ctypes.byref(splits)), "otal_conv_fwd_slabs")
+    _prof_end(ev, "fwd", g)
+    return out, slab.value or 0, splits.value
 
 
 def _conv_forward_half(x, w, k, s, scale, shift, relu, spatial_valid, levels, out):
@@ -967,6 +990,39 @@
     L.check(L.lib().otal_gn_relu_fwd(L.ptr(x), L.ptr(gamma), L.ptr(beta), L.ptr(y), L.ptr(stats), B, C, T, groups,
                                      ctypes.c_float(eps), int(relu), nlev, lev, L.stream()), "otal_gn_relu_fwd")
     return y, stats
+
+
+def _slab_ptr(slab, splits, B, C, T):
+    if isinstance(slab, torch.Tensor):
+        L.require_device(slab)
+        if tuple(slab.shape) != (splits, C, B * T) or slab.dtype != torch.float32:
+            raise RuntimeError(f"slabs have shape {tuple(slab.shape)}, expected {(splits, C, B * T)} float32")
+        return L.ptr(slab)
+    return ctypes.c_void_p(int(slab))
+
+
+def gn_relu_forward_slabs(slab, splits, shift, xout, gamma, beta, groups=32, eps=1e-5, relu=True, levels=None, out=None):
+    L.require_device(xout, gamma, beta)
+    B, C, T = xout.shape
+    nlev, lev = _lev_arg(levels)
+    stats = torch.empty((B, groups, nlev, 2), dtype=torch.float32, device=xout.device)
+    y = torch.empty_like(xout) if out is None else out
+    bs, cs = _dest_strides(y, B, C, T)
+    L.check(L.lib().otal_gn_relu_fwd_slabs(_slab_ptr(slab, splits, B, C, T), int(splits), _opt(shift), L.ptr(xout), L.ptr(gamma),
+                                           L.ptr(beta), L.ptr(y), ctypes.c_int64(bs), ctypes.c_int64(cs), L.ptr(stats), B, C, T,
+                                           groups, ctypes.c_float(eps), int(relu), nlev, lev, L.stream()),
+            "otal_gn_relu_fwd_slabs")
+    return y, stats
+
+
+def conv_gn_relu_forward(x, w, shift, gamma, beta, k, s, groups=32, eps=1e-5, spatial_valid=False, out=None):
+    c, slab, splits = conv_forward_slabs(x, w, k, s, shift=shift, spatial_valid=spatial_valid)
+    c = c.view(c.shape[0], c.shape[1], c.shape[2])
+    if splits > 1:
+        y, st = gn_relu_forward_slabs(slab, splits, shift, c, gamma, beta, groups, eps, True, None, out=out)
+    else:
+        y, st = gn_relu_forward(c, gamma, beta, groups, eps, True, None, out=out)
+    return c, y, st
 
 
 def pyramid_merge_forward(p0, p1, total, up):
@@ -1373,8 +1429,13 @@
         nlev_ = len(levels) - 1
         ctx.scale_params = tensors[:nlev_]
         scales = _adjacent_view(tensors[:nlev_])
+        sptrs = None
         if scales is None:
-            scales = torch.cat([t.detach().reshape(1) for t in tensors[:nlev_]])
+            if all(t.numel() == 1 and t.dtype == torch.float32 and t.is_cuda for t in tensors[:nlev_]):
+                sptrs = (ctypes.c_void_p * nlev_)(*[t.data_ptr() for t in tensors[:nlev_]])
+                scales = tensors[0].detach().new_empty(0)
+            else:
+                scales = torch.cat([t.detach().reshape(1) for t in tensors[:nlev_]])
         raws = [r.contiguous() for r in tensors[nlev_:]]
         L.require_device(scales, *raws)
         B, _, N = raws[0].shape
@@ -1385,9 +1446,13 @@
         arr = lambda ts: VP(*[None if t is None else t.data_ptr() for t in ts])
         strides = None if level_strides is None else (ctypes.c_float * len(level_strides))(*level_strides)
         meta = (L.int_array([r.shape[1] for r in raws]), L.int_array(list(modes)), len(levels) - 1, L.int_array(list(levels)), strides, B, N, n)
-        L.check(L.lib().otal_head_outputs_fwd(n, meta[0], meta[1], arr(raws), arr(outs), arr(uncts), L.ptr(scales), B, N, meta[2],
-                                              meta[3], strides, L.stream()), "otal_head_outputs_fwd")
-        ctx.meta, ctx.modes = meta, tuple(modes)
+        if sptrs is not None:
+            L.check(L.lib().otal_head_outputs_fwd_ptrs(n, meta[0], meta[1], arr(raws), arr(outs), arr(uncts), sptrs, B, N, meta[2],
+                                                       meta[3], strides, L.stream()), "otal_head_outputs_fwd_ptrs")
+        else:
+            L.check(L.lib().otal_head_outputs_fwd(n, meta[0], meta[1], arr(raws), arr(outs), arr(uncts), L.ptr(scales), B, N, meta[2],
+                                                  meta[3], strides, L.stream()), "otal_head_outputs_fwd")
+        ctx.meta, ctx.modes, ctx.scale_ptrs = meta, tuple(modes), sptrs
         ctx.save_for_backward(scales, *raws, *outs, *[u for u in uncts if u is not None])
         return tuple(outs) + tuple(u for u in uncts if u is not None)
 
@@ -1408,18 +1473,30 @@
         VP = ctypes.c_void_p * n
         arr = lambda ts: VP(*[None if t is None else t.data_ptr() for t in ts])
 
+        VL = ctypes.c_void_p * nlev
+        sptrs = ctx.scale_ptrs if ctx.scale_ptrs is not None else VL(*[scales.data_ptr() + 4 * l for l in range(nlev)])
+
         def launch(dscales):
-            L.check(L.lib().otal_head_outputs_bwd(n, chans, modes_a, arr(raws), arr(outs), arr(uncts), arr(douts), arr(dunct), arr(draws),
-                                                  L.ptr(scales), L.ptr(dscales), B, N, nlev, lev, strides, L.stream()),
-                    "otal_head_outputs_bwd")
+            dptrs = VL(*([dscales.data_ptr() + 4 * l for l in range(nlev)] if torch.is_tensor(dscales)
+                         else [t.data_ptr() for t in dscales]))
+            L.check(L.lib().otal_head_outputs_bwd_ptrs(n, chans, modes_a, arr(raws), arr(outs), arr(uncts), arr(douts), arr(dunct),
+                                                       arr(draws), sptrs, dptrs, B, N, nlev, lev, strides, L.stream()),
+                    "otal_head_outputs_bwd_ptrs")
         want = all(ctx.needs_input_grad[3:3 + nlev])
-        slots = [grad_slot(p) if want else None for p in ctx.scale_params]
+        writes = any(m == 1 for m in ctx.modes)
+        if not want:
+            launch(scales.new_empty(nlev))
+            return (None, None, None) + (None,) * nlev + tuple(draws)
+        slots = [grad_slot(p) for p in ctx.scale_params]
+        if writes and all(sl is not None for sl in slots):
+            launch(slots)
+            return (None, None, None) + tuple(slots) + tuple(draws)
         direct = _adjacent_view(slots) if all(sl is not None for sl in slots) else None
         if direct is not None:
             direct.zero_()
             launch(direct)
             return (None, None, None) + tuple(slots) + tuple(draws)
-        dscales = torch.zeros_like(scales)
+        dscales = scales.new_empty(nlev) if writes else scales.new_zeros(nlev)
         launch(dscales)
         if all(sl is not None for sl in slots):
             key = tuple(sl.data_ptr() for sl in slots)
@@ -1633,17 +1710,19 @@
             if not (x.is_cuda and mask.is_cuda) or x.stride(2) != 1 or mask.stride(2) != 1 or x.dtype != torch.float32:
                 raise RuntimeError("boundary losses: float32 GPU maps with unit time stride")
             _, C, T = x.shape
-            if 2 > mask.shape[1] or (T - 1) * step >= mask.shape[2]:
+            if x.shape[0] != B or 2 > mask.shape[1] or (T - 1) * step >= mask.shape[2]:
                 raise RuntimeError("boundary losses: mask rows / length do not cover the map")
-            t = torch.empty((B, 2, T), dtype=torch.float32, device=x.device)
-            dx = torch.empty((B, C, T), dtype=torch.float32, device=x.device)
-            L.check(L.lib().otal_boundary_bce(L.ptr(x), ctypes.c_int64(x.stride(0)), ctypes.c_int64(x.stride(1)), L.ptr(mask),
-                                              ctypes.c_int64(mask.stride(0)), ctypes.c_int64(mask.stride(1)), 0, int(step),
-                                              L.ptr(t), L.ptr(dx), B, C, T, L.stream()), "otal_boundary_bce")
-            terms.append(t); dxs.append(dx)
+            terms.append(torch.empty((B, 2, T), dtype=torch.float32, device=x.device))
+            dxs.append(torch.empty((B, C, T), dtype=torch.float32, device=x.device))
+        VP = lambda ts: (ctypes.c_void_p * n)(*[t.data_ptr() for t in ts])
+        I64 = ctypes.c_int64 * n
+        L.check(L.lib().otal_boundary_bce_multi(n, VP(xs), I64(*[x.stride(0) for x in xs]), I64(*[x.stride(1) for x in xs]),
+                                                L.ptr(mask), ctypes.c_int64(mask.stride(0)), ctypes.c_int64(mask.stride(1)), 0,
+                                                L.int_array([int(s) for s in steps]), VP(terms), VP(dxs), B,
+                                                L.int_array([x.shape[1] for x in xs]), L.int_array([x.shape[2] for x in xs]),
+                                                L.stream()), "otal_boundary_bce_multi")
         out = torch.empty(2, dtype=torch.float32, device=xs[0].device)
         wa = (ctypes.c_float * n)(*[float(w) for w in weights])
-        VP = lambda ts: (ctypes.c_void_p * n)(*[t.data_ptr() for t in ts])
         L.check(L.lib().otal_boundary_finish(n, VP(terms), wa, L.int_array([t.shape[2] for t in terms]), B, L.ptr(out), L.stream()),
                 "otal_boundary_finish")
         ctx.save_for_backward(*dxs)
diff --git a/opental_amd/csrc/bce.hip b/opental_amd/csrc/bce.hip
--- a/opental_amd/csrc/bce.hip
+++ b/opental_amd/csrc/bce.hip
@@ -2,13 +2,12 @@
 
 namespace {
 
-__global__ __launch_bounds__(256) void boundary_bce_kernel(const float* __restrict__ x, int64_t x_bs, int64_t x_cs,
-                                                           const float* __restrict__ mask, int64_t m_bs, int64_t m_rs, int row0,
-                                                           int m_step, float* __restrict__ terms, float* __restrict__ dx,
-                                                           int B, int C, int T) {
-    __shared__ float part[16][17];
+__device__ __forceinline__ void boundary_bce_block(const float* __restrict__ x, int64_t x_bs, int64_t x_cs,
+                                                   const float* __restrict__ mask, int64_t m_bs, int64_t m_rs, int row0,
+                                                   int m_step, float* __restrict__ terms, float* __restrict__ dx,
+                                                   int B, int C, int T, int bx, float (*part)[17]) {
     const int tl = threadIdx.x & 15, cg = threadIdx.x >> 4;
-    const int t = blockIdx.x * 16 + tl, b = blockIdx.y, h = blockIdx.z;
+    const int t = bx * 16 + tl, b = blockIdx.y, h = blockIdx.z;
     const int half = C >> 1;
     const bool live = t < T;
     const float* xp = x + (int64_t)b * x_bs + (int64_t)h * half * x_cs + (live ? t : 0);
@@ -50,6 +49,30 @@
         const float t1 = tanhf(xp[(int64_t)(cg + 16 * i) * x_cs]);
         dp[(int64_t)(cg + 16 * i) * T] = gm * (1.f - t1 * t1);
     }
+}
+
+__global__ __launch_bounds__(256) void boundary_bce_kernel(const float* __restrict__ x, int64_t x_bs, int64_t x_cs,
+                                                           const float* __restrict__ mask, int64_t m_bs, int64_t m_rs, int row0,
+                                                           int m_step, float* __restrict__ terms, float* __restrict__ dx,
+                                                           int B, int C, int T) {
+    __shared__ float part[16][17];
+    boundary_bce_block(x, x_bs, x_cs, mask, m_bs, m_rs, row0, m_step, terms, dx, B, C, T, blockIdx.x, part);
+}
+
+constexpr int BCE_ITEMS = 4;
+struct BceItems {
+    const float* x[BCE_ITEMS]; int64_t x_bs[BCE_ITEMS]; int64_t x_cs[BCE_ITEMS];
+    float* terms[BCE_ITEMS]; float* dx[BCE_ITEMS];
+    int m_step[BCE_ITEMS]; int C[BCE_ITEMS]; int T[BCE_ITEMS]; int start[BCE_ITEMS + 1];
+};
+__global__ __launch_bounds__(256) void boundary_bce_multi_kernel(BceItems it, const float* __restrict__ mask, int64_t m_bs,
+                                                                 int64_t m_rs, int row0, int B) {
+    __shared__ float part[16][17];
+    int i = 0;
+#pragma unroll
+    for (int k = 1; k < BCE_ITEMS; ++k) if ((int)blockIdx.x >= it.start[k]) i = k;
+    boundary_bce_block(it.x[i], it.x_bs[i], it.x_cs[i], mask, m_bs, m_rs, row0, it.m_step[i], it.terms[i], it.dx[i], B, it.C[i],
+                       it.T[i], (int)blockIdx.x - it.start[i], part);
 }
 
 
@@ -116,6 +139,29 @@
     return otal_launch_status();
 }
 
+extern "C" int otal_boundary_bce_multi(int n, const float* const* x, const int64_t* x_batch_stride, const int64_t* x_channel_stride,
+                                       const float* mask, int64_t mask_batch_stride, int64_t mask_row_stride, int mask_row0,
+                                       const int* mask_step, float* const* terms, float* const* dx, int B, const int* C,
+                                       const int* T, void* stream) {
+    if (!x || !x_batch_stride || !x_channel_stride || !mask || !mask_step || !terms || !dx || !C || !T) return OTAL_E_NULL;
+    if (n < 1 || n > BCE_ITEMS || B <= 0 || mask_row0 < 0) return OTAL_E_SHAPE;
+    BceItems it = {};
+    int blocks = 0;
+    for (int i = 0; i < BCE_ITEMS; ++i) {
+        it.start[i] = blocks;
+        if (i >= n) continue;
+        if (!x[i] || !terms[i] || !dx[i]) return OTAL_E_NULL;
+        if (C[i] <= 0 || T[i] <= 0 || (C[i] & 1) || mask_step[i] <= 0) return OTAL_E_SHAPE;
+        it.x[i] = x[i]; it.x_bs[i] = x_batch_stride[i]; it.x_cs[i] = x_channel_stride[i];
+        it.terms[i] = terms[i]; it.dx[i] = dx[i]; it.m_step[i] = mask_step[i]; it.C[i] = C[i]; it.T[i] = T[i];
+        blocks += (T[i] + 15) / 16;
+    }
+    it.start[BCE_ITEMS] = blocks;
+    hipLaunchKernelGGL(boundary_bce_multi_kernel, dim3(blocks, B, 2), dim3(256), 0, (hipStream_t)stream, it, mask,
+                       mask_batch_stride, mask_row_stride, mask_row0, B);
+    return otal_launch_status();
+}
+
 extern "C" int otal_boundary_finish(int n, const float* const* terms, const float* weights, const int* T, int B, float* out2,
                                     void* stream) {
     if (!terms || !weights || !T || !out2) return OTAL_E_NULL;
diff --git a/opental_amd/csrc/conv_gemm.hip b/opental_amd/csrc/conv_gemm.hip
--- a/opental_amd/csrc/conv_gemm.hip
+++ b/opental_amd/csrc/conv_gemm.hip
@@ -1,6 +1,7 @@
 #include "common.h"
 #include "conv_index.h"
 #include "conv_select.h"
+#include "splitk_tree.h"
 #include <cstdlib>
 #include <cstring>
 #include <mutex>
@@ -1807,7 +1808,7 @@
             return 0;
         }
     }
-    if (v4 && a.splits >= 16 && total <= (1 << 21)) {
+    if (splitk_tree_is_tall(total, a.splits, ((uintptr_t)a.slab & 15) == 0)) {
         const int blocks = (int)((total / 4 + 63) / 64);
         hipLaunchKernelGGL((splitk_reduce_tall_kernel<MODE, H>), dim3(blocks), dim3(256), 0, st, a);
         return otal_launch_status();
@@ -2554,6 +2555,9 @@
 #include "conv1x1_stream.inc"
 #endif
 
+struct KeptSlabs { const float* slab; int splits; };
+thread_local KeptSlabs* g_keep_slabs = nullptr;
+
 template <int MODE, bool H = false>
 int launch_chunked(ConvArgs& a, void* ws, size_t ws_bytes, hipStream_t st) {
     const int C = MODE == MODE_FWD ? a.g.Cin : a.g.Cout;
@@ -2633,6 +2637,16 @@
 #undef OTAL_LAUNCH_C
     if (int e = otal_launch_status()) return e;
     if (splits > 1) {
+        if constexpr (!H && MODE == MODE_FWD) {
+            if (g_keep_slabs) {
+                SlabFoldQuery q = {};
+                q.mode = MODE; q.splits = splits;
+                q.spatial = a.g.Ho * a.g.Wo;
+                q.has_scale = a.scale != nullptr; q.relu = (a.flags & EPI_RELU) != 0;
+                q.half = a.half || a.xhalf || a.pair;
+                if (splitk_fold_ok(q)) { g_keep_slabs->slab = a.slab; g_keep_slabs->splits = splits; return 0; }
+            }
+        }
         return launch_splitk_reduce<MODE, H>(a, st);
     }
     return 0;
@@ -2962,6 +2976,46 @@
     }
     if (mode == MODE_DGRAD) front += align256((size_t)g.Cin * g.Cout * kvol * sizeof(float));
     return front + (s > 1 ? (size_t)(s + 1) * M * N * sizeof(float) : 0);
+}
+
+namespace {
+struct KeepScope {
+    explicit KeepScope(KeptSlabs* k) { g_keep_slabs = k; }
+    ~KeepScope() { g_keep_slabs = nullptr; }
+};
+}
+
+extern "C" int otal_conv_fwd_slabs(const int* geom, const int64_t* strides, const float* x, const float* w,
+                                   const float* scale, const float* shift, float* y, int relu, int precision,
+                                   const void* prologue, void* ws, size_t ws_bytes, void* stream,
+                                   const float** slab, int* splits) {
+    if (!slab || !splits) return OTAL_E_NULL;
+    KeptSlabs k = {nullptr, 1};
+    int e;
+    {
+        KeepScope scope(&k);
+        e = otal_conv_fwd(geom, strides, x, w, scale, shift, y, relu, precision, prologue, ws, ws_bytes, stream);
+    }
+    *slab = k.slab; *splits = k.splits;
+    return e;
+}
+
+extern "C" int otal_conv_reduce_slabs(const float* slab, int splits, const float* shift, float* out, int B, int C, int T,
+                                      void* stream) {
+    if (!slab || !out) return OTAL_E_NULL;
+    if (splits < 1 || B <= 0 || C <= 0 || T <= 0) return OTAL_E_SHAPE;
+    if ((int64_t)B * C * T >= (1LL << 31)) return OTAL_E_UNSUPPORTED;
+    ConvArgs a = {};
+    a.g.B = B; a.g.Cin = a.g.Cout = C;
+    a.g.Ti = a.g.To = T; a.g.Hi = a.g.Wi = a.g.Ho = a.g.Wo = 1;
+    a.g.kt = a.g.kh = a.g.kw = 1; a.g.st = a.g.sh = a.g.sw = 1;
+    a.g.x_bs = a.g.y_bs = (int64_t)C * T; a.g.x_cs = a.g.y_cs = T;
+    a.g.nlev = 1;
+    a.fd = make_conv_fastdiv(a.g);
+    a.M = C; a.N = B * T; a.splits = splits;
+    a.slab = const_cast<float*>(slab); a.out = out;
+    a.shift = shift;
+    return launch_splitk_reduce<MODE_FWD>(a, (hipStream_t)stream);
 }
 
 extern "C" int otal_conv_fwd(const int* geom, const int64_t* strides, const float* x, const float* w,
diff --git a/opental_amd/csrc/gn.hip b/opental_amd/csrc/gn.hip
--- a/opental_amd/csrc/gn.hip
+++ b/opental_amd/csrc/gn.hip
@@ -1,4 +1,5 @@
 #include "common.h"
+#include "splitk_tree.h"
 
 namespace {
 
@@ -38,12 +39,35 @@
     }
 }
 
+struct GnSlabs { const float* slab; const float* shift; float* xout; int64_t total; int splits, tall, N; };
+
+__device__ __forceinline__ float slab_sum_seq(const float* __restrict__ p, int64_t total, int s_lo, int s_hi) {
+    float acc = 0.f;
+    for (int s0 = s_lo; s0 < s_hi; s0 += 8) {
+        float tmp[8];
+#pragma unroll
+        for (int u = 0; u < 8; ++u) tmp[u] = p[(int64_t)min(s0 + u, s_hi - 1) * total];
+#pragma unroll
+        for (int u = 0; u < 8; ++u) if (s0 + u < s_hi) acc += tmp[u];
+    }
+    return acc;
+}
+__device__ __forceinline__ float slab_sum(const float* __restrict__ p, int64_t total, int splits, int tall) {
+    if (!tall) return slab_sum_seq(p, total, 0, splits);
+    const int per = (splits + 3) / 4;
+    float q[4];
+#pragma unroll
+    for (int k = 0; k < 4; ++k) q[k] = slab_sum_seq(p, total, k * per, min(splits, k * per + per));
+    return (q[0] + q[1]) + (q[2] + q[3]);
+}
+
 struct GnFwdAlt { const float* x; const float* gamma; const float* beta; float* y; float* stats; };
+template <bool SLAB>
 __global__ __launch_bounds__(256) void gn_relu_fwd_kernel(const float* __restrict__ x, const float* __restrict__ gamma,
                                                           const float* __restrict__ beta, float* __restrict__ y,
                                                           float* __restrict__ stats, int C, int T, int G,
                                                           float eps, int relu, GnLevels L, GnFwdAlt alt,
-                                                          int64_t y_bs, int64_t y_cs) {
+                                                          int64_t y_bs, int64_t y_cs, GnSlabs S) {
     if (blockIdx.y) { x = alt.x; gamma = alt.gamma; beta = alt.beta; y = alt.y; stats = alt.stats; }
     extern __shared__ __attribute__((aligned(16))) char smem[];
     float* buf = reinterpret_cast<float*>(smem);
@@ -58,7 +82,18 @@
     const int n = cpg * T;
     float gv = 0.f, bv = 0.f;
     if (tid < cpg) { gv = gamma[g * cpg + tid]; bv = beta[g * cpg + tid]; }
-    stage_map(buf, x + base, n, tid);
+    if constexpr (SLAB) {
+        for (int i = tid; i < n; i += 256) {
+            const int c = i / T, t = i - c * T;
+            const int ch = g * cpg + c;
+            float v = slab_sum(S.slab + (int64_t)ch * S.N + (int64_t)b * T + t, S.total, S.splits, S.tall);
+            if (S.shift) v += S.shift[ch];
+            buf[i] = v;
+            S.xout[base + i] = v;
+        }
+    } else {
+        stage_map(buf, x + base, n, tid);
+    }
     if (tid < cpg) { gam[tid] = gv; bet[tid] = bv; }
     __syncthreads();
     if (L.nlev == 1) {
@@ -276,9 +311,9 @@
     const size_t lds = (size_t)(C / G) * T * 4 + 64 + (size_t)(C / G) * 8;
     if (lds > LDS_MAX) return OTAL_E_UNSUPPORTED;
     static bool large_ok = false;
-    if (int e = allow_large_lds(gn_relu_fwd_kernel, lds, large_ok)) return e;
-    hipLaunchKernelGGL(gn_relu_fwd_kernel, dim3(B * G), dim3(256), lds, (hipStream_t)stream,
-                       x, gamma, beta, y, stats, C, T, G, eps, relu, L, GnFwdAlt{}, (int64_t)C * T, (int64_t)T);
+    if (int e = allow_large_lds(gn_relu_fwd_kernel<false>, lds, large_ok)) return e;
+    hipLaunchKernelGGL(gn_relu_fwd_kernel<false>, dim3(B * G), dim3(256), lds, (hipStream_t)stream,
+                       x, gamma, beta, y, stats, C, T, G, eps, relu, L, GnFwdAlt{}, (int64_t)C * T, (int64_t)T, GnSlabs{});
     return otal_layer_launched("gn_relu_fwd<single>");
 }
 
@@ -293,9 +328,9 @@
     const size_t lds = (size_t)(C / G) * T * 4 + 64 + (size_t)(C / G) * 8;
     if (lds > LDS_MAX) return OTAL_E_UNSUPPORTED;
     static bool large_ok = false;
-    if (int e = allow_large_lds(gn_relu_fwd_kernel, lds, large_ok)) return e;
-    hipLaunchKernelGGL(gn_relu_fwd_kernel, dim3(B * G), dim3(256), lds, (hipStream_t)stream,
-                       x, gamma, beta, y, stats, C, T, G, eps, relu, L, GnFwdAlt{}, y_bs, y_cs);
+    if (int e = allow_large_lds(gn_relu_fwd_kernel<false>, lds, large_ok)) return e;
+    hipLaunchKernelGGL(gn_relu_fwd_kernel<false>, dim3(B * G), dim3(256), lds, (hipStream_t)stream,
+                       x, gamma, beta, y, stats, C, T, G, eps, relu, L, GnFwdAlt{}, y_bs, y_cs, GnSlabs{});
     return otal_layer_launched("gn_relu_fwd<single>");
 }
 
@@ -311,8 +346,8 @@
     const size_t lds = (size_t)(C / G) * T * 4 + 64 + (size_t)(C / G) * 8;
     if (lds > 64 * 1024) return OTAL_E_UNSUPPORTED;
     const GnFwdAlt alt = {x[1], gamma[1], beta[1], y[1], stats[1]};
-    hipLaunchKernelGGL(gn_relu_fwd_kernel, dim3(B * G, 2), dim3(256), lds, (hipStream_t)stream,
-                       x[0], gamma[0], beta[0], y[0], stats[0], C, T, G, eps, relu, L, alt, (int64_t)C * T, (int64_t)T);
+    hipLaunchKernelGGL(gn_relu_fwd_kernel<false>, dim3(B * G, 2), dim3(256), lds, (hipStream_t)stream,
+                       x[0], gamma[0], beta[0], y[0], stats[0], C, T, G, eps, relu, L, alt, (int64_t)C * T, (int64_t)T, GnSlabs{});
     return otal_layer_launched("gn_relu_fwd<pair>");
 }
 
@@ -328,8 +363,8 @@
     const size_t lds = (size_t)(C / G) * T * 4 + 64 + (size_t)(C / G) * 8;
     if (lds > 64 * 1024) return OTAL_E_UNSUPPORTED;
     const GnFwdAlt alt = {x[1], gamma[1], beta[1], y[1], stats[1]};
-    hipLaunchKernelGGL(gn_relu_fwd_kernel, dim3(B * G, 2), dim3(256), lds, (hipStream_t)stream,
-                       x[0], gamma[0], beta[0], y[0], stats[0], C, T, G, eps, relu, L, alt, y_bs, y_cs);
+    hipLaunchKernelGGL(gn_relu_fwd_kernel<false>, dim3(B * G, 2), dim3(256), lds, (hipStream_t)stream,
+                       x[0], gamma[0], beta[0], y[0], stats[0], C, T, G, eps, relu, L, alt, y_bs, y_cs, GnSlabs{});
     return otal_layer_launched("gn_relu_fwd<pair>");
 }
 
@@ -409,6 +444,37 @@
 }
 
 namespace {
+int fill_slabs(GnSlabs& S, const float* slab, int splits, int B, int C, int T) {
+    const int64_t total = (int64_t)B * C * T;
+    if (!slab) return OTAL_E_NULL;
+    if (splits < 1 || total >= (1LL << 31)) return OTAL_E_SHAPE;
+    S.slab = slab; S.total = total; S.splits = splits; S.N = B * T;
+    S.tall = splitk_tree_is_tall(total, splits, (reinterpret_cast<uintptr_t>(slab) & 15) == 0) ? 1 : 0;
+    return 0;
+}
+}
+
+extern "C" int otal_gn_relu_fwd_slabs(const float* slab, int splits, const float* shift, float* xout, const float* gamma,
+                                      const float* beta, float* y, int64_t y_bs, int64_t y_cs, float* stats, int B, int C, int T,
+                                      int G, float eps, int relu, int nlev, const int* lev, void* stream) {
+    g_layer_kernel = "";
+    if (!slab || !xout || !gamma || !beta || !y || !stats) return OTAL_E_NULL;
+    if (B <= 0 || C <= 0 || T <= 0 || G <= 0 || C % G || y_cs < T || y_bs < 0) return OTAL_E_SHAPE;
+    GnLevels L;
+    if (int e = fill_levels(L, T, nlev, lev)) return e;
+    GnSlabs S = {};
+    if (int e = fill_slabs(S, slab, splits, B, C, T)) return e;
+    S.shift = shift; S.xout = xout;
+    const size_t lds = (size_t)(C / G) * T * 4 + 64 + (size_t)(C / G) * 8;
+    if (lds > LDS_MAX) return OTAL_E_UNSUPPORTED;
+    static bool large_ok = false;
+    if (int e = allow_large_lds(gn_relu_fwd_kernel<true>, lds, large_ok)) return e;
+    hipLaunchKernelGGL(gn_relu_fwd_kernel<true>, dim3(B * G), dim3(256), lds, (hipStream_t)stream,
+                       nullptr, gamma, beta, y, stats, C, T, G, eps, relu, L, GnFwdAlt{}, y_bs, y_cs, S);
+    return otal_layer_launched(S.tall ? "gn_relu_fwd<slabs,tall>" : "gn_relu_fwd<slabs>");
+}
+
+namespace {
 constexpr int SP_MAX = 32;
 struct SumItems { const float* src[SP_MAX]; float* dst[SP_MAX][3]; int C[SP_MAX]; int B[SP_MAX]; };
 __global__ __launch_bounds__(256) void sum_partials_kernel(const SumItems it) {
diff --git a/opental_amd/csrc/heads.hip b/opental_amd/csrc/heads.hip
--- a/opental_amd/csrc/heads.hip
+++ b/opental_amd/csrc/heads.hip
@@ -15,7 +15,7 @@
     const float* dunct[MAX_ITEMS];
     float* draw[MAX_ITEMS];
 };
-struct HeadLevels { int nlev; int lev[OTAL_MAX_LEVELS + 1]; float stride[OTAL_MAX_LEVELS]; };
+struct HeadLevels { int nlev; int lev[OTAL_MAX_LEVELS + 1]; float stride[OTAL_MAX_LEVELS]; const float* sp[OTAL_MAX_LEVELS]; float* dsp[OTAL_MAX_LEVELS]; };
 
 __device__ __forceinline__ int level_of(const HeadLevels& L, int n) {
     int l = 0;
@@ -25,7 +25,7 @@
     return l;
 }
 
-__global__ __launch_bounds__(256) void heads_fwd_kernel(HeadItems it, HeadLevels L, const float* __restrict__ scales, int B, int N) {
+__global__ __launch_bounds__(256) void heads_fwd_kernel(HeadItems it, HeadLevels L, int B, int N) {
     const int n = blockIdx.x * 256 + threadIdx.x, b = blockIdx.y, i = blockIdx.z;
     if (n >= N) return;
     const int C = it.C[i], mode = it.mode[i];
@@ -33,7 +33,7 @@
     float* y = it.out[i] + ((size_t)b * N + n) * C;
     if (mode == 1) {
         const int l = level_of(L, n);
-        const float s = scales[l], f = L.stride[l];
+        const float s = *L.sp[l], f = L.stride[l];
         for (int c = 0; c < C; ++c) y[c] = expf(x[(size_t)c * N] * s) * f;
         return;
     }
@@ -47,8 +47,7 @@
     if (mode >= 2) it.unct[i][(size_t)b * N + n] = (float)C / sum;
 }
 
-__global__ __launch_bounds__(256) void heads_bwd_kernel(HeadItems it, HeadLevels L, const float* __restrict__ scales,
-                                                        float* __restrict__ dscales, int B, int N) {
+__global__ __launch_bounds__(256) void heads_bwd_kernel(HeadItems it, HeadLevels L, int B, int N) {
     const int i = blockIdx.z;
     if (i == it.n_items) {
         if (blockIdx.x != 0 || blockIdx.y != 0) return;
@@ -70,7 +69,7 @@
                 if (threadIdx.x < s) red[threadIdx.x] += red[threadIdx.x + s];
                 __syncthreads();
             }
-            if (threadIdx.x == 0) dscales[l] = red[0];
+            if (threadIdx.x == 0) *L.dsp[l] = red[0];
             __syncthreads();
         }
         return;
@@ -81,7 +80,7 @@
     float* dx = it.draw[i] + (size_t)b * C * N + n;
     const float* dy = it.dout[i] ? it.dout[i] + ((size_t)b * N + n) * C : nullptr;
     if (mode == 1) {
-        const float s = scales[level_of(L, n)];
+        const float s = *L.sp[level_of(L, n)];
         const float* y = it.out[i] + ((size_t)b * N + n) * C;
         for (int c = 0; c < C; ++c) dx[(size_t)c * N] = dy ? dy[c] * y[c] * s : 0.f;
         return;
@@ -121,28 +120,48 @@
 
 }
 
+namespace {
+int heads_fwd(int n_items, const int* channels, const int* modes, const float* const* raw, float* const* out, float* const* unct,
+              const float* scales, const float* const* scale_ptrs, int B, int N, int nlev, const int* lev,
+              const float* level_strides, void* stream) {
+    if (!channels || !modes || !raw || !out || !unct) return OTAL_E_NULL;
+    HeadItems it;
+    HeadLevels L = {};
+    if (int e = fill(it, L, n_items, channels, modes, B, N, nlev, lev, level_strides)) return e;
+    bool have = scales || scale_ptrs;
+    for (int l = 0; l < nlev; ++l) {
+        L.sp[l] = scale_ptrs ? scale_ptrs[l] : (scales ? scales + l : nullptr);
+        have = have && L.sp[l];
+    }
+    for (int i = 0; i < n_items; ++i) {
+        if (!raw[i] || !out[i] || (modes[i] >= 2 && !unct[i]) || (modes[i] == 1 && !have)) return OTAL_E_NULL;
+        it.raw[i] = raw[i]; it.out[i] = out[i]; it.unct[i] = unct[i];
+    }
+    hipLaunchKernelGGL(heads_fwd_kernel, dim3((N + 255) / 256, B, n_items), dim3(256), 0, (hipStream_t)stream, it, L, B, N);
+    return otal_launch_status();
+}
+}
+
 extern "C" int otal_head_outputs_fwd(int n_items, const int* channels, const int* modes, const float* const* raw, float* const* out,
                                      float* const* unct, const float* scales, int B, int N, int nlev, const int* lev,
                                      const float* level_strides, void* stream) {
-    if (!channels || !modes || !raw || !out || !unct) return OTAL_E_NULL;
-    HeadItems it;
-    HeadLevels L;
-    if (int e = fill(it, L, n_items, channels, modes, B, N, nlev, lev, level_strides)) return e;
-    for (int i = 0; i < n_items; ++i) {
-        if (!raw[i] || !out[i] || (modes[i] >= 2 && !unct[i]) || (modes[i] == 1 && !scales)) return OTAL_E_NULL;
-        it.raw[i] = raw[i]; it.out[i] = out[i]; it.unct[i] = unct[i];
-    }
-    hipLaunchKernelGGL(heads_fwd_kernel, dim3((N + 255) / 256, B, n_items), dim3(256), 0, (hipStream_t)stream, it, L, scales, B, N);
-    return otal_launch_status();
-}
-
-extern "C" int otal_head_outputs_bwd(int n_items, const int* channels, const int* modes, const float* const* raw,
-                                     const float* const* out, const float* const* unct, const float* const* dout,
-                                     const float* const* dunct, float* const* draw, const float* scales, float* dscales, int B,
-                                     int N, int nlev, const int* lev, const float* level_strides, void* stream) {
+    return heads_fwd(n_items, channels, modes, raw, out, unct, scales, nullptr, B, N, nlev, lev, level_strides, stream);
+}
+
+extern "C" int otal_head_outputs_fwd_ptrs(int n_items, const int* channels, const int* modes, const float* const* raw,
+                                          float* const* out, float* const* unct, const float* const* scale_ptrs, int B, int N,
+                                          int nlev, const int* lev, const float* level_strides, void* stream) {
+    return heads_fwd(n_items, channels, modes, raw, out, unct, nullptr, scale_ptrs, B, N, nlev, lev, level_strides, stream);
+}
+
+namespace {
+int heads_bwd(int n_items, const int* channels, const int* modes, const float* const* raw, const float* const* out,
+              const float* const* unct, const float* const* dout, const float* const* dunct, float* const* draw,
+              const float* scales, float* dscales, const float* const* scale_ptrs, float* const* dscale_ptrs, int B, int N,
+              int nlev, const int* lev, const float* level_strides, void* stream) {
     if (!channels || !modes || !raw || !out || !unct || !dout || !dunct || !draw) return OTAL_E_NULL;
     HeadItems it;
-    HeadLevels L;
+    HeadLevels L = {};
     if (int e = fill(it, L, n_items, channels, modes, B, N, nlev, lev, level_strides)) return e;
     bool any_exp = false;
     for (int i = 0; i < n_items; ++i) {
@@ -151,8 +170,33 @@
         it.dout[i] = dout[i]; it.dunct[i] = dunct[i]; it.draw[i] = draw[i];
         any_exp = any_exp || modes[i] == 1;
     }
-    if (any_exp && (!scales || !dscales)) return OTAL_E_NULL;
+    bool have = true;
+    for (int l = 0; l < nlev; ++l) {
+        L.sp[l] = scale_ptrs ? scale_ptrs[l] : (scales ? scales + l : nullptr);
+        L.dsp[l] = dscale_ptrs ? dscale_ptrs[l] : (dscales ? dscales + l : nullptr);
+        have = have && L.sp[l] && L.dsp[l];
+    }
+    if (any_exp && !have) return OTAL_E_NULL;
     hipLaunchKernelGGL(heads_bwd_kernel, dim3((N + 255) / 256, B, n_items + (any_exp ? 1 : 0)), dim3(256), 0, (hipStream_t)stream,
-                       it, L, scales, dscales, B, N);
+                       it, L, B, N);
     return otal_launch_status();
 }
+}
+
+extern "C" int otal_head_outputs_bwd(int n_items, const int* channels, const int* modes, const float* const* raw,
+                                     const float* const* out, const float* const* unct, const float* const* dout,
+                                     const float* const* dunct, float* const* draw, const float* scales, float* dscales, int B,
+                                     int N, int nlev, const int* lev, const float* level_strides, void* stream) {
+    return heads_bwd(n_items, channels, modes, raw, out, unct, dout, dunct, draw, scales, dscales, nullptr, nullptr, B, N, nlev, lev,
+                     level_strides, stream);
+}
+
+extern "C" int otal_head_outputs_bwd_ptrs(int n_items, const int* channels, const int* modes, const float* const* raw,
+                                          const float* const* out, const float* const* unct, const float* const* dout,
+                                          const float* const* dunct, float* const* draw, const float* const* scale_ptrs,
+                                          float* const* dscale_ptrs, int B, int N, int nlev, const int* lev,
+                                          const float* level_strides, void* stream) {
+    if (!scale_ptrs || !dscale_ptrs) return OTAL_E_NULL;
+    return heads_bwd(n_items, channels, modes, raw, out, unct, dout, dunct, draw, nullptr, nullptr, scale_ptrs, dscale_ptrs, B, N,
+                     nlev, lev, level_strides, stream);
+}
diff --git a/opental_amd/csrc/splitk_tree.h b/opental_amd/csrc/splitk_tree.h
--- /dev/null
+++ b/opental_amd/csrc/splitk_tree.h
@@ -0,0 +1,23 @@
+#pragma once
+#include <stdint.h>
+
+namespace {
+
+static inline bool splitk_tree_is_tall(int64_t total, int splits, bool slab_aligned16) {
+    const bool v4 = (total % 4 == 0) && slab_aligned16;
+    return v4 && splits >= 16 && total <= (1 << 21);
+}
+
+struct SlabFoldQuery {
+    int mode;
+    int splits;
+    int spatial;
+    int has_scale, relu, half;
+};
+static inline bool splitk_fold_ok(const SlabFoldQuery& q) {
+    if (q.splits < 2) return false;
+    if (q.spatial != 1 || q.half) return false;
+    return q.mode == 0 && !q.has_scale && !q.relu;
+}
+
+}
diff --git a/opental_amd/thumos14/pyramid_fused.py b/opental_amd/thumos14/pyramid_fused.py
--- a/opental_amd/thumos14/pyramid_fused.py
+++ b/opental_amd/thumos14/pyramid_fused.py
@@ -115,10 +115,10 @@
         tape = {}
         early = ops.STEP.early_results.pop(x1.data_ptr(), None)
         if early is None:
-            c0 = ops.conv_forward(x1, pyr[0][0], cfg["k0"], ONE, shift=pyr[0][1], spatial_valid=True).view(B, C, t0)
-            p0, st0 = ops.gn_relu_forward(c0, pyr[0][2], pyr[0][3], G, eps, True, None)
-        c1 = ops.conv_forward(x2, pyr[1][0], cfg["k1"], ONE, shift=pyr[1][1], spatial_valid=True).view(B, C, t0 // 2)
-        p1, st1 = ops.gn_relu_forward(c1, pyr[1][2], pyr[1][3], G, eps, True, None)
+            c0, p0, st0 = ops.conv_gn_relu_forward(x1, pyr[0][0], pyr[0][1], pyr[0][2], pyr[0][3], cfg["k0"], ONE, G, eps,
+                                                   spatial_valid=True)
+        c1, p1, st1 = ops.conv_gn_relu_forward(x2, pyr[1][0], pyr[1][1], pyr[1][2], pyr[1][3], cfg["k1"], ONE, G, eps,
+                                               spatial_valid=True)
         if early is not None:
             c0, p0, st0, elane = early
             elane.join()
@@ -143,8 +143,8 @@
         ptape = []
         for l in range(2, len(lev) - 1):
             x = packed[:, :, lev[l - 1]:lev[l]]
-            c = ops.conv_forward(x, pyr[l][0], K3, S2, shift=pyr[l][1])
-            _, st = ops.gn_relu_forward(c, pyr[l][2], pyr[l][3], G, eps, True, None, out=packed[:, :, lev[l]:lev[l + 1]])
+            c, _, st = ops.conv_gn_relu_forward(x, pyr[l][0], pyr[l][1], pyr[l][2], pyr[l][3], K3, S2, G, eps,
+                                                out=packed[:, :, lev[l]:lev[l + 1]])
             ptape.append((c, st))
         s1 = _conv_gn_pair((packed, packed), (lt[0], ct[0]), K3, lev, G, eps)
         s2 = _conv_gn_pair((s1[0][1], s1[1][1]), (lt[1], ct[1]), K3, lev, G, eps)
```

After: 1020, median of 6. Within noise of the previous version (+0.7%).
